# trifectatechfoundation/zlib-rs

Hardware: NVIDIA H100
Metric: deflate_level6_raw_input_throughput_silesia_small_tar (higher is better)
Workload: dtype u8

## Files before the change

zlib_rs_b200/csrc/zb_engine.cu:

```cuda
#include <cuda_runtime.h>
#include <stdio.h>
#include <stdlib.h>
#include <string.h>
#include <algorithm>
#include <cassert>
#include <new>
#include "../../include/zb_engine.h"
#include "zb_kernels.cuh"
#include "zb_engine_internal.h"

namespace zb {

constexpr uint32_t kSlowSub9 = 24576;
constexpr uint32_t kTailTiles = 2;
constexpr uint32_t kTailSub = 512;

thread_local char g_err[256] = "";

static void set_err(const char *what, cudaError_t e)
{
    snprintf(g_err, sizeof g_err, "%s: %s", what, cudaGetErrorString(e));
}

#define CK(call)                                                  \
    do {                                                          \
        cudaError_t e_ = (call);                                  \
        if (e_ != cudaSuccess) { set_err(#call, e_); return ZB_E_CUDA; } \
    } while (0)

__global__ void k_match(JobBufs);
__global__ void k_skip(JobBufs, uint32_t);
__global__ void k_skip_walk(JobBufs);
__global__ void k_nxt(JobBufs);
__global__ void k_path_tiles(JobBufs);
__global__ void k_path_chain(JobBufs, uint32_t, uint32_t);
__global__ void k_path_groups(JobBufs, uint32_t, uint32_t, uint4 *, uint32_t *);
__global__ void k_path_chain2(JobBufs, uint32_t, uint32_t, const uint4 *, uint32_t *, uint32_t *);
__global__ void k_path_mark(JobBufs, const uint32_t *, const uint32_t *);
__global__ void k_iter_lists(JobBufs, uint32_t *, uint32_t *, uint32_t);
__global__ void k_emit(JobBufs);
__global__ void k_holes(JobBufs, uint32_t);
__global__ void k_holes_cmp(JobBufs, uint32_t, uint32_t);
__global__ void k_tail(JobBufs);
__global__ void k_block_hist(JobBufs, uint32_t *);
__global__ void k_build_blocks(JobBufs, const uint32_t *);
__global__ void k_scan_blocks(JobBufs);
__global__ void k_encode(JobBufs);
__global__ void k_finish(JobBufs, const uint32_t *);
__global__ void k_literal_syms(JobBufs);
__global__ void k_stored(JobBufs);
__global__ void k_links2_std(JobBufs, uint32_t);
__global__ void k_links2_roll(JobBufs, uint32_t);
__global__ void k_links_fix_std(JobBufs);
__global__ void k_links_fix_roll(JobBufs);
__global__ void k_slow(JobBufs);
__global__ void k_rle(JobBufs);
__global__ void k_emit_slow(JobBufs);
__global__ void k_tail_slow(JobBufs);
__global__ void k_serial_low(JobBufs);
__global__ void k_links_dict_ghost(JobBufs, uint32_t *);
__global__ void k_links_dict_ghost_apply(JobBufs, const uint32_t *);
__global__ void k_bgzf_setup(BgzfJob, uint64_t);
__global__ void k_serial_low_members(JobBufs, BgzfJob);
__global__ void k_bgzf_medium(JobBufs, BgzfJob);
__global__ void k_bgzf_slow_steps(JobBufs, BgzfJob);
__global__ void k_bgzf_slow_walk(JobBufs, BgzfJob);
__global__ void k_bgzf_rle_steps(JobBufs, BgzfJob);
__global__ void k_bgzf_literals(JobBufs, BgzfJob);
__global__ void k_bgzf_hist(JobBufs, BgzfJob, uint32_t *);
__global__ void k_bgzf_build(JobBufs, BgzfJob, const uint32_t *);
__global__ void k_bgzf_size(JobBufs, BgzfJob);
__global__ void k_bgzf_scan(JobBufs, BgzfJob);
__global__ void k_bgzf_encode(JobBufs, BgzfJob);
__global__ void k_bgzf_frame(JobBufs, BgzfJob);
__global__ void k_batch_stage(const uint8_t *, const uint64_t *, const uint8_t *, const uint64_t *, BgzfJob, uint8_t *, uint64_t);
__global__ void k_batch_dict_ghost(JobBufs, BgzfJob);
__global__ void k_flush_blocks(JobBufs, BgzfJob);
__global__ void k_deflate_points(JobBufs, BgzfJob, IdxWriteJob);

constexpr uint32_t kMatchSmemBytes = (kWSize + kMatchSub + 512) + (kWSize + kMatchSub) * 2 + ((kWSize + kMatchSub) / 32 + 1) * 4 * 4 + 8192;
constexpr uint32_t kPathSmemBytes = kPathTile * 4 * 3;
constexpr uint32_t kLinks2SmemBytes = 65536 * 2 + kLinkTile * 2 + kLinkTile + 64 + 2048;
constexpr uint32_t kSkipSmemBytes = 2 * kWSize * 2 + 2 * (2 * kWSize / 32) * 4 + 8192 + 64;
constexpr uint32_t kSkipWalkSmemBytes = (kWSize + kSkipSlice) * 2 + (kWSize + kSkipSlice) / 32 * 4 + 8192;
constexpr uint32_t kSlowSubMax = 24576;
constexpr uint32_t kSlowSmemBytes = (kWSize + kSlowSubMax + kSlowAhead) * 3;
constexpr uint32_t kChainSmemBytes = kChainChunkTiles * kPathHead * 8;
constexpr uint32_t kChain2MaxSmem = 200 * 1024;
constexpr uint32_t kSerialSmemBytes = (65536 + kWSize) * 2 + 35824 + 16;
constexpr uint32_t kSerialSmemQuick = 65536 * 2 + 65536 + 16;

int Engine::init(int dev)
{
    int n = 0;
    cudaError_t e = cudaGetDeviceCount(&n);
    if (e != cudaSuccess || n == 0) {
        snprintf(g_err, sizeof g_err, "no CUDA device (%s)", e == cudaSuccess ? "count 0" : cudaGetErrorString(e));
        return ZB_E_NODEVICE;
    }
    if (dev < 0 || dev >= n) { snprintf(g_err, sizeof g_err, "device %d out of range", dev); return ZB_E_PARAM; }
    device = dev;
    CK(cudaSetDevice(dev));
    CK(cudaStreamCreateWithFlags(&st, cudaStreamNonBlocking));
    CK(cudaStreamCreateWithFlags(&st2, cudaStreamNonBlocking));
    CK(cudaEventCreateWithFlags(&evf, cudaEventDisableTiming));
    CK(cudaEventCreateWithFlags(&evt, cudaEventDisableTiming));
    for (int i = 0; i < kUpChunks; i++) CK(cudaEventCreateWithFlags(&evc[i], cudaEventDisableTiming));
    CK(cudaEventCreateWithFlags(&evk, cudaEventDisableTiming));
    CK(cudaEventCreate(&ev0));
    CK(cudaEventCreate(&ev1));
    CK(upload_tables());
    CK(cudaFuncSetAttribute(k_match, cudaFuncAttributeMaxDynamicSharedMemorySize, kMatchSmemBytes));
    CK(cudaFuncSetAttribute(k_skip, cudaFuncAttributeMaxDynamicSharedMemorySize, kSkipSmemBytes));
    CK(cudaFuncSetAttribute(k_skip_walk, cudaFuncAttributeMaxDynamicSharedMemorySize, kSkipWalkSmemBytes));
    CK(cudaFuncSetAttribute(k_links2_std, cudaFuncAttributeMaxDynamicSharedMemorySize, kLinks2SmemBytes));
    CK(cudaFuncSetAttribute(k_links2_roll, cudaFuncAttributeMaxDynamicSharedMemorySize, kLinks2SmemBytes));
    CK(cudaFuncSetAttribute(k_slow, cudaFuncAttributeMaxDynamicSharedMemorySize, kSlowSmemBytes));
    CK(cudaFuncSetAttribute(k_path_tiles, cudaFuncAttributeMaxDynamicSharedMemorySize, kPathSmemBytes));
    CK(cudaFuncSetAttribute(k_path_mark, cudaFuncAttributeMaxDynamicSharedMemorySize, kPathSmemBytes));
    CK(cudaFuncSetAttribute(k_path_chain, cudaFuncAttributeMaxDynamicSharedMemorySize, kChainSmemBytes));
    CK(cudaFuncSetAttribute(k_path_groups, cudaFuncAttributeMaxDynamicSharedMemorySize, kChain2MaxSmem));
    CK(cudaFuncSetAttribute(k_path_chain2, cudaFuncAttributeMaxDynamicSharedMemorySize, kChain2MaxSmem));
    CK(cudaFuncSetAttribute(k_serial_low, cudaFuncAttributeMaxDynamicSharedMemorySize, kSerialSmemBytes));
    CK(cudaFuncSetAttribute(k_serial_low_members, cudaFuncAttributeMaxDynamicSharedMemorySize, kSerialSmemBytes));
    CK(cudaMallocHost(&h_info, sizeof(JobInfo)));
    CK(cudaMalloc(&d_info, sizeof(JobInfo)));
    CK(cudaMalloc(&d_check, 16));
    { int rc_ = inflate_init(); if (rc_ != ZB_OK) return rc_; }
    return ZB_OK;
}

Engine::~Engine()
{
    if (device < 0) return;
    cudaSetDevice(device);
    for (auto &b : bufs) if (b.p) cudaFree(b.p);
    if (h_stage) cudaFreeHost(h_stage);
    if (h_info) cudaFreeHost(h_info);
    if (d_info) cudaFree(d_info);
    if (d_check) cudaFree(d_check);
    if (ev0) cudaEventDestroy(ev0);
    if (ev1) cudaEventDestroy(ev1);
    if (evf) cudaEventDestroy(evf);
    if (evt) cudaEventDestroy(evt);
    for (int i = 0; i < kUpChunks; i++) if (evc[i]) cudaEventDestroy(evc[i]);
    if (evk) cudaEventDestroy(evk);
    if (st2) cudaStreamDestroy(st2);
    if (st) cudaStreamDestroy(st);
}

void Engine::pbegin()
{
    if (!profile) return;
    if (!pev0) { cudaEventCreate(&pev0); cudaEventCreate(&pev1); }
    cudaEventRecord(pev0, st);
}

void Engine::pend(int phase, uint32_t nlaunch)
{
    if (!profile) return;
    cudaEventRecord(pev1, st);
    cudaEventSynchronize(pev1);
    float ms = 0;
    cudaEventElapsedTime(&ms, pev0, pev1);
    phase_ms[phase] += ms;
    phase_launches[phase] += nlaunch;
}

int Engine::reserve(int slot, size_t bytes, void **out)
{
    Buf &b = bufs[slot];
    if (b.cap < bytes) {
        if (b.p) { cudaFree(b.p); b.p = nullptr; b.cap = 0; }
        size_t want = bytes + (bytes >> 3) + 4096;
        cudaError_t e = cudaMalloc(&b.p, want);
        if (e != cudaSuccess) { set_err("cudaMalloc", e); return ZB_E_MEM; }
        b.cap = want;
    }
    *out = b.p;
    return ZB_OK;
}

int Engine::stage(size_t bytes)
{
    if (h_stage_cap < bytes) {
        if (h_stage) cudaFreeHost(h_stage);
        h_stage = nullptr;
        h_stage_cap = 0;
        cudaError_t e = cudaMallocHost(&h_stage, bytes + (bytes >> 3) + 4096);
        if (e != cudaSuccess) { set_err("cudaMallocHost", e); return ZB_E_MEM; }
        h_stage_cap = bytes + (bytes >> 3) + 4096;
    }
    return ZB_OK;
}


size_t deflate_bound(size_t n) { return (size_t)stream_bound(n); }

int Engine::deflate(const void *src, size_t n_in, bool src_dev, void *dst, size_t dst_cap, bool dst_dev, int level, int strategy,
                    int window_bits, uint32_t flags, zb_deflate_result *res, const void *dict, size_t dict_len, IdxWrite *iw)
{
    if (flags & ZB_FLAG_BGZF) {
        const uint32_t ml = (flags >> 8) & 15u;
        if ((flags & ~(ZB_FLAG_BGZF | ZB_FLAG_MEMLEVEL(15))) || (ml && ml != 8) || dict_len || window_bits != 31 || strategy != 0 ||
            level < -1 || level > 9) {
            snprintf(g_err, sizeof g_err, "ZB_FLAG_BGZF takes window_bits 31, Z_DEFAULT_STRATEGY, level -1..9 and no other flag");
            return ZB_E_PARAM;
        }
        return deflate_bgzf(src, n_in, src_dev, dst, dst_cap, dst_dev, level, res, iw);
    }
    size_t dstart = 0;
    if (dict_len) {
        if (!dict || window_bits >= 0) { snprintf(g_err, sizeof g_err, "a dictionary needs a raw stream (the caller frames FDICT / DICTID)"); return ZB_E_PARAM; }
        if (dict_len >= 2 * (size_t)kWSize) { dict = static_cast<const uint8_t *>(dict) + (dict_len - kWSize); dict_len = kWSize; }
        dstart = dict_len;
    }
    const size_t n = n_in + dstart;
    int mem_level = (int)((flags >> 8) & 15u);
    if (mem_level == 0) mem_level = 8;
    if (mem_level > 9) return ZB_E_PARAM;
    if (!res || (!src && n) || !dst) return ZB_E_PARAM;
    memset(res, 0, sizeof *res);
    if (n > 0xF0000000ull) { snprintf(g_err, sizeof g_err, "input too large for one job (%zu)", n); return ZB_E_PARAM; }
    if (level == -1) level = 6;
    if (level < 0 || level > 9 || strategy < 0 || strategy > 4) return ZB_E_PARAM;
    uint32_t wrap;
    if (window_bits < 0) { if (window_bits < -15 || window_bits > -8) return ZB_E_PARAM; wrap = 0; }
    else if (window_bits > 15) { if (window_bits < 24 || window_bits > 31) return ZB_E_PARAM; wrap = 2; }
    else { if (window_bits < 8) return ZB_E_PARAM; wrap = 1; }
    const int wb = window_bits < 0 ? -window_bits : window_bits > 15 ? window_bits - 16 : window_bits;
    CK(cudaSetDevice(device));
    const uint32_t N = (uint32_t)n;
    launches = 0;

    JobBufs jb;
    memset(&jb, 0, sizeof jb);
    int rc;
    void *p;
    const size_t npad = (size_t)N + kPad;
    const uint32_t nwords = (N >> 5) + 2;
    const uint32_t nmt = N / kMatchTile + 1, npt = N / kPathTile + 1;
    const bool low_parallel = (flags & ZB_FLAG_LOW_PARALLEL) != 0 || dstart != 0;
    const bool serial_low = (level == 1 || level == 2) && strategy != 2 && strategy != 3 && !low_parallel;
    const uint32_t block_syms = (serial_low && level == 1) ? kBlockSyms : (1u << (mem_level + 6)) - 1u;
    const uint32_t max_blocks = N / block_syms + 2;
    const size_t out_cap = (deflate_bound(n) + 15) & ~(size_t)15;
    if ((rc = stage((size_t)nmt + 64 + ((size_t)N / 512 + 2 + npt + nmt + 8) * 4 + 64)) != ZB_OK) return rc;
    uint8_t *h_dirty = static_cast<uint8_t *>(h_stage);
    uint32_t *h_lists = reinterpret_cast<uint32_t *>(static_cast<uint8_t *>(h_stage) + (((size_t)nmt + 64 + 15) & ~(size_t)15));
#define RES(slot, bytes, field, type)                                   \
    if ((rc = reserve(slot, bytes, &p)) != ZB_OK) return rc;            \
    jb.field = static_cast<type>(p);
    uint8_t *d_in;
    if ((rc = reserve(S_IN, npad + 16, &p)) != ZB_OK) return rc;
    d_in = static_cast<uint8_t *>(p);
    jb.in = d_in;
    jb.N = N;
    jb.start = (uint32_t)dstart;
    jb.nmt = nmt;
    jb.tail_start = N > 2 * kTailZone ? N - kTailZone : 0;
    jb.block_syms = block_syms;
    jb.serial_mode = serial_low ? (uint32_t)level : 0u;
    RES(S_L, npad * 2, L, uint16_t *)
    RES(S_SK, npad * 2, SK, uint16_t *)
    RES(S_HOLES, (size_t)nwords * 4, holes, uint32_t *)
    RES(S_HOLESN, (size_t)nwords * 4, holes_new, uint32_t *)
    RES(S_M, npad * 4, M, uint32_t *)
    RES(S_NXT, ((size_t)N + 16) * 4, nxt, uint32_t *)
    RES(S_PEXIT, ((size_t)N + 16) * 4, pexit, uint32_t *)
    RES(S_PCNT, ((size_t)N + 16) * 4, pcnt, uint32_t *)
    RES(S_SYMIDX, ((size_t)N + 16) * 4, symidx, uint32_t *)
    RES(S_PHEAD, (size_t)npt * kPathHead * 8, phead, uint2 *)
    RES(S_TENTRY, (size_t)npt * 4, tile_entry, uint32_t *)
    RES(S_TSYMB, (size_t)npt * 4, tile_symbase, uint32_t *)
    RES(S_MARKN, (size_t)npt + 16, mark_needed, uint8_t *)
    const uint32_t nlists = npt * (kPathTile / kPathSub);
    RES(S_LLIST, (size_t)nlists * kLongPerSub * 4, long_list, uint32_t *)
    RES(S_LCNT, (size_t)nlists * 4, long_cnt, uint32_t *)
    RES(S_TDIRTY, 2 * ((size_t)nmt + 16), tile_dirty, uint8_t *)
    jb.skip_fall = jb.tile_dirty + nmt + 16;
    RES(S_SYMS, ((size_t)N + 64) * sizeof(Sym), syms, Sym *)
    RES(S_SYMB, 40000 * 4, sym_base, uint32_t *)
    RES(S_BMAP, (size_t)nmt * 8192, bucket_map, uint32_t *)
    RES(S_LR, npad * 2, Lr, uint16_t *)
    RES(S_KEYS, npad * 2, keys, uint16_t *)
    RES(S_LLAST, (size_t)nmt * 65536 * 2, link_last, uint16_t *)
    RES(S_CSTATE, (size_t)(npt + 1) * 16, chain_state, uint4 *)
    uint32_t chainG = 16;
    while ((uint64_t)chainG * chainG < npt) chainG += 8;
    const uint32_t chain_groups = (npt + chainG - 1) / chainG;
    const uint32_t chain2_smem = chainG * kPathHead * 8 + chain_groups * kPathHead * 16 + chainG * 8;
    const bool chain2 = chain2_smem <= kChain2MaxSmem;
    if ((rc = reserve(S_GFN, (size_t)chain_groups * kPathHead * 16 + ((size_t)npt + 4) * 4, &p)) != ZB_OK) return rc;
    uint4 *d_gfn = static_cast<uint4 *>(p);
    uint32_t *d_mark_cnt = reinterpret_cast<uint32_t *>(d_gfn + (size_t)chain_groups * kPathHead);
    uint32_t *d_mark_list = d_mark_cnt + 4;
    auto launch_chain = [&](uint32_t first_tile) {
        if (chain2) {
            k_path_groups<<<chain_groups, 1024, chainG * kPathHead * 8, st>>>(jb, npt, chainG, d_gfn, d_mark_cnt);
            k_path_chain2<<<chain_groups, 1024, chain2_smem, st>>>(jb, npt, chainG, d_gfn, d_mark_list, d_mark_cnt);
            launches++;
        } else k_path_chain<<<1, 1024, kChainSmemBytes, st>>>(jb, npt, first_tile);
    };
    auto launch_mark = [&](uint32_t grid) {
        if (chain2) k_path_mark<<<grid < npt ? grid : npt, 1024, kPathSmemBytes, st>>>(jb, d_mark_list, d_mark_cnt);
        else k_path_mark<<<npt, 1024, kPathSmemBytes, st>>>(jb, nullptr, nullptr);
    };
    uint32_t *d_lists;
    const uint32_t max_list = N / 512 + 2;
    if ((rc = reserve(S_LISTS, ((size_t)max_list + npt + nmt + 8) * 4, &p)) != ZB_OK) return rc;
    d_lists = static_cast<uint32_t *>(p);
    RES(S_HDIFF, (size_t)nwords * 8, hdiff, uint32_t *)
    jb.hdiff_words = nwords;
    RES(S_HCOARSE, (size_t)(N >> 10) + 16, hcoarse, uint8_t *)
    RES(S_MCHG, (((size_t)N >> 8) + 16) * 4 + 64, mchg, uint8_t *)
    RES(S_BLOCKS, (size_t)max_blocks * sizeof(BlockDesc), blocks, BlockDesc *)
    RES(S_BBASE, (size_t)max_blocks * 4, block_base, uint32_t *)
    uint32_t *d_freq;
    if ((rc = reserve(S_FREQ, (size_t)max_blocks * 320 * 4, &p)) != ZB_OK) return rc;
    d_freq = static_cast<uint32_t *>(p);
    uint8_t *d_out;
    if (dst_dev && dst_cap >= out_cap) d_out = static_cast<uint8_t *>(dst);
    else { if ((rc = reserve(S_OUT, out_cap + 16, &p)) != ZB_OK) return rc; d_out = static_cast<uint8_t *>(p); }
    jb.out = d_out;
    jb.out_cap = out_cap;
    void *d_ck;
    const size_t ck_bytes = ((size_t)N / 16384 + 16) * 8;
    if ((rc = reserve(S_CK, ck_bytes, &d_ck)) != ZB_OK) return rc;
#undef RES
    jb.info = d_info;
    jb.level = (uint32_t)level;
    jb.strategy_fixed = strategy == 4;
    const bool lf_zero = strategy >= 2;
    jb.wrap = wrap;
    jb.hdr_len = wrap == 1 ? 2 : wrap == 2 ? 10 : 0;
    jb.huffman_only = strategy == 2 && level != 0;
    jb.not_last = (flags & ZB_FLAG_NOT_LAST) ? 1 : 0;
    jb.end_mode = (flags & ZB_FLAG_END_PARTIAL) ? 1u : (flags & ZB_FLAG_END_BLOCK) ? 2u : 0u;
    jb.prime_bits = (flags >> 12) & 7u;
    if ((jb.end_mode && !jb.not_last) || (jb.prime_bits && wrap != 0)) { snprintf(g_err, sizeof g_err, "END_* needs NOT_LAST, PRIME a raw stream"); return ZB_E_PARAM; }
    if (jb.not_last && (level == 0 || wrap != 0)) { snprintf(g_err, sizeof g_err, "NOT_LAST needs raw deflate and level > 0"); return ZB_E_PARAM; }
    jb.xfl = gzip_xfl(level, strategy);
    int eng_level = level;
    const int wb_eff = wb == 8 ? 9 : wb;
    const bool small_ok = wb_eff < 15 && (uint64_t)N + kMinLookahead <= (1ull << wb_eff);
    bool exact = (wb_eff == 15 || small_ok) && (dstart == 0 || wb_eff == 15);
    jb.cinfo = small_ok ? (uint32_t)(wb_eff - 8) : 7u;
    jb.wsize = kWSize;
    const bool serial_win = wb_eff < 15 && !small_ok && N <= 32000u && level >= 3 && level <= 6 && strategy != 2 && strategy != 3;
    if (serial_win) {
        jb.wsize = 1u << wb_eff;
        jb.cinfo = (uint32_t)(wb_eff - 8);
        jb.tail_start = 0;
        exact = true;
    }
    const bool par_win = wb_eff < 15 && !small_ok && !serial_win && level >= 3 && level <= 6 && strategy != 2 && strategy != 3 && dstart == 0;
    if (par_win) {
        jb.wsize = 1u << wb_eff;
        jb.cinfo = (uint32_t)(wb_eff - 8);
        exact = true;
    }
    const bool slow_win = wb_eff < 15 && !small_ok && dstart == 0 && level != 0 && ((level >= 7 && strategy != 2) || strategy == 3);
    if (slow_win) {
        jb.wsize = 1u << wb_eff;
        jb.cinfo = (uint32_t)(wb_eff - 8);
        exact = true;
    }
    if (wb_eff < 15 && (level == 0 || (strategy == 2 && level != 0) || serial_low)) {
        jb.wsize = 1u << wb_eff;
        jb.cinfo = (uint32_t)(wb_eff - 8);
        exact = true;
    }
    if (level != 0 && !jb.huffman_only) {
        if (level < 3 && !serial_low) { eng_level = 3; exact = exact && strategy == 3; }
        if (strategy == 3) jb.slow_mode = 2;
        else if (level > 6) { jb.slow_mode = 1; jb.sp = slow_params(level); jb.sp.filtered = strategy == 1; jb.sp.wsize = jb.wsize; }
    }
    if (jb.slow_mode) jb.tail_start = N;
    jb.lp = level_params(eng_level);
    if (level != 0 && !jb.huffman_only) jb.level = (uint32_t)level;
    if (lf_zero && !jb.strategy_fixed && !jb.huffman_only) jb.level = 1;

    CK(cudaEventRecord(ev0, st));
    if (profile) { for (int i = 0; i < kPhases; i++) { phase_ms[i] = 0; phase_launches[i] = 0; } }
    uint32_t up_chunks = 0;
    size_t up_len[kUpChunks] = {0};
    const bool chunked_upload = !src_dev && !dstart && n_in >= ((size_t)4 << 20) && level != 0 && !jb.huffman_only &&
                                !jb.serial_mode && jb.slow_mode != 2;
    if (chunked_upload) {
        size_t chunk = ((n_in + kUpChunks - 1) / kUpChunks + kLinkTile - 1) / kLinkTile * kLinkTile;
        if (chunk < (size_t)device_sm_count() * kLinkTile) chunk = (size_t)device_sm_count() * kLinkTile;
        CK(cudaStreamWaitEvent(st2, ev0, 0));
        for (size_t off = 0; off < n_in; off += chunk) {
            const size_t len = n_in - off < chunk ? n_in - off : chunk;
            CK(cudaMemcpyAsync(d_in + off, static_cast<const uint8_t *>(src) + off, len, cudaMemcpyHostToDevice, st2));
            if (off + len == n_in) CK(cudaMemsetAsync(d_in + n, 0, kPad, st2));
            CK(cudaEventRecord(evc[up_chunks], st2));
            up_len[up_chunks++] = off + len;
        }
    } else {
        pbegin();
        if (dstart) CK(cudaMemcpyAsync(d_in, dict, dstart, src_dev ? cudaMemcpyDefault : cudaMemcpyHostToDevice, st));
        if (n_in) CK(cudaMemcpyAsync(d_in + dstart, src, n_in, src_dev ? cudaMemcpyDeviceToDevice : cudaMemcpyHostToDevice, st));
        CK(cudaMemsetAsync(d_in + n, 0, kPad, st));
        pend(9, 0);
    }
    CK(cudaMemsetAsync(d_info, 0, sizeof(JobInfo), st));
    CK(cudaMemsetAsync(d_out, 0, out_cap, st));
    if (jb.prime_bits) {
        h_prime = (uint8_t)((flags >> 16) & ((1u << jb.prime_bits) - 1u));
        CK(cudaMemcpyAsync(d_out, &h_prime, 1, cudaMemcpyHostToDevice, st));
    }
    cudaStream_t st_ck = chunked_upload ? st2 : st;
    pbegin();
    if (wrap == 1 || (wrap == 0 && (flags & ZB_FLAG_CHECK_ADLER))) { CK(launch_adler32(d_in + dstart, n_in, 1, d_ck, ck_bytes, d_check, st_ck)); launches += 2; }
    else if (wrap == 2 || (wrap == 0 && (flags & ZB_FLAG_CHECK_CRC))) { CK(launch_crc32(d_in + dstart, n_in, 0, d_ck, ck_bytes, d_check, st_ck)); launches += 2; }
    else CK(cudaMemsetAsync(d_check, 0, 4, st_ck));
    if (chunked_upload) CK(cudaEventRecord(evk, st2));
    pend(8, 2);

    auto links_tiles = [&](bool roll) {
        uint32_t t_done = 0;
        for (uint32_t k = 0; k < (chunked_upload ? up_chunks : 1u); k++) {
            uint32_t t_hi = nmt;
            if (chunked_upload) {
                cudaStreamWaitEvent(st, evc[k], 0);
                if (k + 1 < up_chunks) t_hi = up_len[k] >= 64 ? (uint32_t)((up_len[k] - 64) / kLinkTile) : 0;
            }
            if (t_hi <= t_done) continue;
            if (roll) k_links2_roll<<<t_hi - t_done, 1024, kLinks2SmemBytes, st>>>(jb, t_done);
            else k_links2_std<<<t_hi - t_done, 1024, kLinks2SmemBytes, st>>>(jb, t_done);
            if (k) launches++;
            t_done = t_hi;
        }
        if (chunked_upload) cudaStreamWaitEvent(st, evk, 0);
    };
    uint32_t iters = 0;
    if (level == 0) {
        const uint32_t nb = n_in == 0 ? 1 : (uint32_t)((n_in + 65534) / 65535);
        k_stored<<<nb, 256, 0, st>>>(jb);
        launches++;
        k_finish<<<1, 32, 0, st>>>(jb, d_check);
        launches++;
    } else {
        if (jb.huffman_only) {
            k_literal_syms<<<(uint32_t)(n_in / 256 + 1), 256, 0, st>>>(jb);
            launches++;
        } else if (jb.serial_mode) {
            iters = 1;
            pbegin();
            k_serial_low<<<1, 32, jb.serial_mode == 2 ? kSerialSmemBytes : kSerialSmemQuick, st>>>(jb);
            launches++;
            pend(1, 1);
        } else {
            CK(cudaMemsetAsync(jb.holes, 0, (size_t)nwords * 4, st));
            CK(cudaMemsetAsync(jb.holes_new, 0, (size_t)nwords * 4, st));
            CK(cudaMemsetAsync(jb.tile_dirty, 1, nmt, st));
            CK(cudaMemsetAsync(jb.skip_fall, 0, nmt, st));
            CK(cudaMemsetAsync(jb.tile_entry, 0xee, (size_t)npt * 4, st));
            CK(cudaMemsetAsync(jb.M + N, 0, (size_t)kPad * 4, st));
            CK(cudaMemsetAsync(jb.L + N, 0, (size_t)kPad * 2, st));
            pbegin();
            if (jb.slow_mode == 2) {
            } else if (jb.slow_mode && jb.sp.slow) {
                links_tiles(true);
                k_links_fix_roll<<<N / 256 + 1, 256, 0, st>>>(jb);
                launches += 2;
            } else {
                links_tiles(false);
                k_links_fix_std<<<N / 256 + 1, 256, 0, st>>>(jb);
                launches += 2;
                if (dstart >= 3 && n_in) {
                    uint32_t *d_first = reinterpret_cast<uint32_t *>(d_check) + 2;
                    CK(cudaMemsetAsync(d_first, 0xff, 4, st));
                    k_links_dict_ghost<<<(kMaxDist + 255) / 256, 256, 0, st>>>(jb, d_first);
                    k_links_dict_ghost_apply<<<1, 32, 0, st>>>(jb, d_first);
                    launches += 2;
                }
            }
            if (!jb.slow_mode) CK(cudaMemcpyAsync(jb.Lr, jb.L, npad * 2, cudaMemcpyDeviceToDevice, st));
            pend(0, 1);
            if (jb.slow_mode) {
                if (n_in > 0) {
                    iters = 1;
                    pbegin();
                    if (jb.slow_mode == 2) k_rle<<<(N + 255) / 256, 256, 0, st>>>(jb);
                    else {
                        jb.match_sub = level >= 9 ? kSlowSub9 : level == 8 ? 4096u : 8192u;
                        k_slow<<<(N + jb.match_sub - 1) / jb.match_sub, 1024, (kWSize + jb.match_sub + kSlowAhead) * 3, st>>>(jb);
                    }
                    pend(1, 1);
                    if (profile) phase_ms[11] = phase_ms[1];
                    pbegin();
                    k_path_tiles<<<npt, 1024, kPathSmemBytes, st>>>(jb);
                    launch_chain(0);
                    launch_mark(npt);
                    pend(3, 3);
                    pbegin();
                    k_emit_slow<<<(N + 255) / 256, 256, 0, st>>>(jb);
                    pend(4, 1);
                    launches += 5;
                }
                pbegin();
                k_tail_slow<<<1, 32, 0, st>>>(jb);
                launches++;
                pend(5, 1);
            } else {
            if (jb.tail_start > 0) {
                uint32_t n_dirty = nmt;
                for (;;) {
                    iters++;
                    uint32_t mthreads = 1024;
                    if (iters == 1) jb.match_sub = 4096;
                    else if (n_dirty <= kTailTiles) { jb.match_sub = kTailSub; mthreads = 256; }
                    else {
                        const uint64_t per_cta = (uint64_t)n_dirty * kMatchTile / (4 * (uint64_t)device_sm_count());
                        jb.match_sub = per_cta >= 8192 ? 8192 : per_cta >= 4096 ? 4096 : per_cta >= 2048 ? 2048 : 1024;
                    }
                    uint32_t nsub = (N + jb.match_sub - 1) / jb.match_sub;
                    uint32_t n_ptiles = npt, first_ptile = 0;
                    jb.skip_list = nullptr;
                    jb.nxt_list = nullptr;
                    if (iters > 1) {
                        jb.skip_list = d_lists;
                        jb.nxt_list = d_lists + nmt + 8;
                        n_ptiles = h_info->n_ptiles ? h_info->n_ptiles : 1;
                        first_ptile = h_info->first_ptile;
                        nsub = (n_dirty ? n_dirty : 1) * (kMatchTile / jb.match_sub);
                        if (n_dirty > kSkipWalkTiles) {
                            pbegin();
                            k_skip<<<n_dirty, 1024, kSkipSmemBytes, st>>>(jb, 0);
                            pend(1, 1);
                            launches++;
                        } else if (n_dirty) {
                            pbegin();
                            k_skip_walk<<<n_dirty * (kMatchTile / kSkipSlice), 1024, kSkipWalkSmemBytes, st>>>(jb);
                            k_skip<<<n_dirty, 1024, kSkipSmemBytes, st>>>(jb, 1);
                            pend(1, 2);
                            launches += 2;
                        }
                    }
                    const uint32_t msmem = (kWSize + jb.match_sub + 512) + (kWSize + jb.match_sub) * 2 +
                                           (iters > 1 ? ((kWSize + jb.match_sub) / 32 + 1) * 4 * 4 + 8192 : 64);
                    jb.use_bucket_map = iters > 1;
                    pbegin();
                    k_match<<<nsub, mthreads, msmem, st>>>(jb);
                    pend(1, 1);
                    if (profile && iters == 1) phase_ms[11] = phase_ms[1];
                    pbegin();
                    k_nxt<<<n_ptiles * (kPathTile / 1024), 1024, 0, st>>>(jb);
                    pend(2, 1);
                    pbegin();
                    k_path_tiles<<<n_ptiles, 1024, kPathSmemBytes, st>>>(jb);
                    launch_chain(first_ptile);
                    launch_mark(iters == 1 ? npt : 2 * n_ptiles + 16);
                    pend(3, 3);
                    pbegin();
                    k_holes<<<(nlists * kLongPerSub + 255) / 256, 256, 0, st>>>(jb, nlists);
                    k_holes_cmp<<<(nwords + 255) / 256, 256, 0, st>>>(jb, nwords, nmt);
                    pend(4, 2);
                    launches += 7;
                    k_iter_lists<<<1, 1024, 0, st>>>(jb, d_lists, d_lists + nmt + 8, npt);
                    launches++;
                    CK(cudaMemcpyAsync(h_info, d_info, sizeof(JobInfo), cudaMemcpyDeviceToHost, st));
                    CK(cudaStreamSynchronize(st));
                    if (h_info->error) { snprintf(g_err, sizeof g_err, "engine error flags 0x%x (parse)", h_info->error); return ZB_E_INTERNAL; }
                    if (getenv("ZB_DEBUG")) {
                        static unsigned long long last[3];
                        if (iters == 1) memset(last, 0, sizeof last);
                        const double ctas = (double)(h_info->dbg[0] - last[0]) + 1e-9;
                        fprintf(stderr, "iter %u dirty %u: ctas %llu stage %.1f walk %.1f kcyc/cta, holes_changed %u, sub %u first_tile %u chain %u\n",
                                iters, n_dirty, h_info->dbg[0] - last[0], (h_info->dbg[1] - last[1]) / 1e3 / ctas,
                                (h_info->dbg[2] - last[2]) / 1e3 / ctas, h_info->holes_changed, jb.match_sub, first_ptile, chain2 ? 2u : 1u);
                        memcpy(last, h_info->dbg, sizeof last);
                    }
                    if (!h_info->holes_changed) break;
                    n_dirty = h_info->n_dirty;
                    if (iters > N / 257u + 4096u) { snprintf(g_err, sizeof g_err, "hole iteration did not converge"); return ZB_E_INTERNAL; }
                }
            }
            CK(cudaEventRecord(evf, st));
            CK(cudaStreamWaitEvent(st2, evf, 0));
            k_tail<<<1, 32, 0, st2>>>(jb);
            launches++;
            CK(cudaEventRecord(evt, st2));
            if (jb.tail_start > 0) {
                pbegin();
                k_emit<<<(jb.tail_start + 255) / 256, 256, 0, st>>>(jb);
                launches++;
                pend(4, 1);
            }
            pbegin();
            CK(cudaStreamWaitEvent(st, evt, 0));
            pend(5, 1);
            }
        }
        CK(cudaMemcpyAsync(h_info, d_info, sizeof(JobInfo), cudaMemcpyDeviceToHost, st));
        CK(cudaStreamSynchronize(st));
        if (h_info->error) { snprintf(g_err, sizeof g_err, "engine error flags 0x%x (tail)", h_info->error); return ZB_E_INTERNAL; }
        const uint32_t nblocks = h_info->n_blocks;
        if (nblocks == 0 || nblocks > max_blocks) { snprintf(g_err, sizeof g_err, "bad block count %u", nblocks); return ZB_E_INTERNAL; }
        pbegin();
        k_block_hist<<<nblocks, 256, 0, st>>>(jb, d_freq);
        k_build_blocks<<<nblocks, 32, 0, st>>>(jb, d_freq);
        k_scan_blocks<<<1, 256, 0, st>>>(jb);
        pend(6, 3);
        pbegin();
        k_encode<<<nblocks, 1024, 0, st>>>(jb);
        k_finish<<<1, 32, 0, st>>>(jb, d_check);
        pend(7, 2);
        launches += 5;
    }
    CK(cudaMemcpyAsync(h_info, d_info, sizeof(JobInfo), cudaMemcpyDeviceToHost, st));
    CK(cudaStreamSynchronize(st));
    CK(cudaGetLastError());
    if (h_info->error) {
        if (h_info->error & 8u) return ZB_E_BUF;
        snprintf(g_err, sizeof g_err, "engine error flags 0x%x (encode)", h_info->error);
        return ZB_E_INTERNAL;
    }
    const uint64_t out_bytes = h_info->out_bytes;
    if (out_bytes > dst_cap) {
        res->out_bytes = out_bytes;
        return ZB_E_BUF;
    }
    if (iw) {
        IdxWriteJob w{iw->span, zbi_targets(n, iw->span), n, 1, 0, level == 0 ? 1u : 0u, 0, nullptr, nullptr};
        const IdxHeader h{kIdxMagic, kIdxVersion, iw->span, n, out_bytes, wrap ? h_info->adler : 1u, wrap == 0 ? -15 : wrap == 1 ? 15 : 31,
                          0, 0, 0};
        BgzfJob bj;
        memset(&bj, 0, sizeof bj);
        if ((rc = index_written(jb, bj, w, h, iw)) != ZB_OK) return rc;
    }
    if (d_out != dst) {
        pbegin();
        CK(cudaMemcpyAsync(dst, d_out, out_bytes, dst_dev ? cudaMemcpyDeviceToDevice : cudaMemcpyDeviceToHost, st));
        pend(10, 0);
    }
    CK(cudaEventRecord(ev1, st));
    CK(cudaStreamSynchronize(st));
    float ms = 0;
    CK(cudaEventElapsedTime(&ms, ev0, ev1));
    res->out_bytes = out_bytes;
    res->check = h_info->adler;
    res->data_type = (int32_t)h_info->data_type;
    res->iterations = iters;
    res->n_symbols = h_info->n_syms;
    res->n_blocks = h_info->n_blocks;
    res->gpu_launches = launches;
    res->exact_parity = exact ? 1 : 0;
    res->gpu_ms = ms;
    res->bits_used = (uint32_t)(h_info->total_bits & 7u) ? (uint32_t)(h_info->total_bits & 7u) : 8u;
    if (jb.not_last && jb.end_mode && (h_info->total_bits & 7u)) {
        uint8_t last = 0;
        CK(cudaMemcpy(&last, d_out + out_bytes, 1, cudaMemcpyDeviceToHost));
        res->carry = last & ((1u << (h_info->total_bits & 7u)) - 1u);
    }
    return ZB_OK;
}

MemberClasses MemberClasses::uniform(int level, uint32_t nm, uint32_t N)
{
    MemberParams mp;
    batch_member_params(level, 0 , 15, 8, 0, &mp);
    MemberClasses mc;
    mc.level = level;
    mc.nslots = level > 0 ? nm * kBgzfMaxBlocks : 0u;
    for (uint32_t c = mp.cls + 1; c <= kClasses; c++) {
        mc.beg[c] = nm;
        mc.off[c] = N;
    }
    return mc;
}

int Engine::members_alloc(JobBufs &jb, BgzfJob &bj, const MemberClasses &mc, uint32_t nm, uint32_t S, size_t span, size_t out_cap,
                          uint32_t wrap, uint32_t **d_freq)
{
    const uint32_t nmt = S / kLinkTile + 1, nslots = mc.nslots;
    memset(&jb, 0, sizeof jb);
    bj = BgzfJob{};
    int rc;
    void *p;
#define RES(slot, bytes, field, type)                                   \
    if ((rc = reserve(slot, bytes, &p)) != ZB_OK) return rc;            \
    jb.field = static_cast<type>(p);
    RES(S_IN, span + kPad + 16, in, const uint8_t *)
    jb.N = S;
    jb.wsize = kWSize;
    RES(S_OUT, out_cap + 16, out, uint8_t *)
    jb.out_cap = out_cap;
    *d_freq = nullptr;
    if (nslots) {
        RES(S_SYMS, (span + 64) * sizeof(Sym), syms, Sym *)
        RES(S_BLOCKS, (size_t)nslots * sizeof(BlockDesc), blocks, BlockDesc *)
        RES(S_BBASE, (size_t)nslots * 4, block_base, uint32_t *)
        if ((rc = reserve(S_FREQ, (size_t)nslots * 320 * 4, &p)) != ZB_OK) return rc;
        *d_freq = static_cast<uint32_t *>(p);
    }
    if (mc.any(kClassMedium, kClassRle)) {
        RES(S_L, (span + kPad) * 2, L, uint16_t *)
        RES(S_KEYS, (span + kPad) * 2, keys, uint16_t *)
        RES(S_LLAST, (size_t)nmt * 65536 * 2, link_last, uint16_t *)
    }
    if (mc.any(kClassSlow, kClassHuff)) {
        RES(S_M, span * 4, M, uint32_t *)
        RES(S_NXT, span * 4, nxt, uint32_t *)
    }
#undef RES
    const size_t m8 = ((size_t)nm * 8 + 15) & ~(size_t)15, m4 = ((size_t)nm * 4 + 15) & ~(size_t)15;
    const size_t mi_bytes = ((size_t)nm * sizeof(JobInfo) + 15) & ~(size_t)15;
    if ((rc = reserve(S_BGZF, 2 * m8 + 4 * m4 + mi_bytes + sizeof(BgzfCtl), &p)) != ZB_OK) return rc;
    uint8_t *t = static_cast<uint8_t *>(p);
    bj.nm = nm;
    bj.wrap = wrap;
    bj.moff = reinterpret_cast<uint64_t *>(t);
    bj.mout = reinterpret_cast<uint64_t *>(t + m8);
    bj.mlen = reinterpret_cast<uint32_t *>(t + 2 * m8);
    bj.mcheck = reinterpret_cast<uint32_t *>(t + 2 * m8 + m4);
    bj.mbytes = reinterpret_cast<uint32_t *>(t + 2 * m8 + 2 * m4);
    bj.mstored = reinterpret_cast<uint32_t *>(t + 2 * m8 + 3 * m4);
    bj.minfo = reinterpret_cast<JobInfo *>(t + 2 * m8 + 4 * m4);
    bj.ctl = reinterpret_cast<BgzfCtl *>(t + 2 * m8 + 4 * m4 + mi_bytes);
    if (mc.level >= 0) {
        const int level = mc.level;
        jb.level = (uint32_t)level;
        jb.block_syms = kBlockSyms;
        jb.serial_mode = level == 1 || level == 2 ? (uint32_t)level : 0u;
        if (level >= 3 && level <= 6) jb.lp = level_params(level);
        if (level >= 7) { jb.slow_mode = 1; jb.sp = slow_params(level); jb.sp.wsize = kWSize; }
    }
    return ZB_OK;
}

static size_t result_bytes(const BgzfJob &bj)
{
    return reinterpret_cast<const uint8_t *>(bj.ctl + 1) - reinterpret_cast<const uint8_t *>(bj.minfo);
}

int Engine::members_stage(const JobBufs &jb, const BgzfJob &bj, const uint64_t *h_moff, const uint32_t *h_mlen, const uint64_t *h_soff,
                          uint64_t *d_soff, size_t n_soff, const void *src, bool src_dev, uint64_t base, uint64_t total, uint8_t *d_copy,
                          const uint8_t *d_dict, const uint64_t *d_mdsrc)
{
    const uint32_t nm = bj.nm;
    CK(cudaMemcpyAsync(bj.moff, h_moff, (size_t)nm * 8, cudaMemcpyHostToDevice, st));
    CK(cudaMemcpyAsync(bj.mlen, h_mlen, (size_t)nm * 4, cudaMemcpyHostToDevice, st));
    CK(cudaMemcpyAsync(d_soff, h_soff, n_soff * 8, cudaMemcpyHostToDevice, st));
    if (!src_dev && total) CK(cudaMemcpyAsync(d_copy, static_cast<const uint8_t *>(src) + base, total, cudaMemcpyHostToDevice, st));
    const uint8_t *d_src = src_dev ? static_cast<const uint8_t *>(src) + base : d_copy;
    k_batch_stage<<<nm, 256, 0, st>>>(d_src + (h_soff[0] - base), d_soff, d_dict, d_mdsrc, bj, const_cast<uint8_t *>(jb.in), jb.N);
    CK(cudaMemsetAsync(const_cast<uint8_t *>(jb.in) + jb.N, 0, kPad + 16, st));
    CK(cudaMemsetAsync(bj.minfo, 0, result_bytes(bj), st));
    CK(cudaMemsetAsync(jb.out, 0, jb.out_cap, st));
    launches++;
    return ZB_OK;
}

void Engine::members_parse(const JobBufs &jb, const BgzfJob &bj, const MemberClasses &mc, bool ghost)
{
    auto links = [&](uint32_t c0, uint32_t c1, bool roll) {
        if (!mc.any(c0, c1)) return false;
        JobBufs r = jb;
        r.in += mc.off[c0];
        r.L += mc.off[c0];
        r.keys += mc.off[c0];
        r.N = (uint32_t)(mc.off[c1] - mc.off[c0]);
        const uint32_t nt = r.N / kLinkTile + 1;
        if (roll) {
            k_links2_roll<<<nt, 1024, kLinks2SmemBytes, st>>>(r, 0);
            k_links_fix_roll<<<r.N / 256 + 1, 256, 0, st>>>(r);
        } else {
            k_links2_std<<<nt, 1024, kLinks2SmemBytes, st>>>(r, 0);
            k_links_fix_std<<<r.N / 256 + 1, 256, 0, st>>>(r);
        }
        launches += 2;
        return true;
    };
    auto view = [&](uint32_t c0, uint32_t c1) {
        const uint32_t m0 = mc.beg[c0];
        assert(m0 == 0 || bj.mslot);
        const auto at = [m0](auto *t) { return t ? t + m0 : t; };
        BgzfJob v = bj;
        v.nm = mc.beg[c1] - m0;
        v.moff = at(v.moff);
        v.mlen = at(v.mlen);
        v.minfo = at(v.minfo);
        v.mp = at(v.mp);
        v.mslot = at(v.mslot);
        v.mps = at(v.mps);
        v.mdx = at(v.mdx);
        return v;
    };
    if (links(kClassMedium, kClassSlow9, false) && ghost) {
        const BgzfJob v = view(kClassMedium, kClassSlow9);
        k_batch_dict_ghost<<<v.nm, 256, 0, st>>>(jb, v);
        launches++;
    }
    links(kClassSlow9, kClassRle, true);
    if (mc.any(kClassQuick, kClassQuick + 1)) {
        JobBufs q = jb;
        q.serial_mode = 1;
        const BgzfJob v = view(kClassQuick, kClassQuick + 1);
        k_serial_low_members<<<v.nm, 32, kSerialSmemQuick, st>>>(q, v);
        launches++;
    }
    if (mc.any(kClassFast, kClassFast + 1)) {
        JobBufs q = jb;
        q.serial_mode = 2;
        const BgzfJob v = view(kClassFast, kClassFast + 1);
        k_serial_low_members<<<v.nm, 32, kSerialSmemBytes, st>>>(q, v);
        launches++;
    }
    if (mc.any(kClassMedium, kClassMedium + 1)) {
        const BgzfJob v = view(kClassMedium, kClassMedium + 1);
        k_bgzf_medium<<<v.nm, 32, 0, st>>>(jb, v);
        launches++;
    }
    if (mc.any(kClassSlow, kClassRle)) {
        const BgzfJob v = view(kClassSlow, kClassRle);
        k_bgzf_slow_steps<<<v.nm * (kMemberMax / 256), 256, 0, st>>>(jb, v);
        k_bgzf_slow_walk<<<(v.nm + 31) / 32, 32, 0, st>>>(jb, v);
        launches += 2;
    }
    if (mc.any(kClassRle, kClassRle + 1)) {
        const BgzfJob v = view(kClassRle, kClassRle + 1);
        k_bgzf_rle_steps<<<v.nm * (kMemberMax / 256), 256, 0, st>>>(jb, v);
        k_bgzf_slow_walk<<<(v.nm + 31) / 32, 32, 0, st>>>(jb, v);
        launches += 2;
    }
    if (mc.any(kClassHuff, kClassHuff + 1)) {
        const BgzfJob v = view(kClassHuff, kClassHuff + 1);
        k_bgzf_literals<<<v.nm * (kMemberMax / 256), 256, 0, st>>>(jb, v);
        launches++;
    }
    if (bj.flushed && mc.any(kClassFast, kClasses)) { k_flush_blocks<<<bj.nm / 256 + 1, 256, 0, st>>>(jb, bj); launches++; }
}

int Engine::members_blocks(JobBufs &jb, BgzfJob &bj, uint32_t nslots, uint32_t *d_freq)
{
    const uint32_t nm = bj.nm;
    if (nslots) {
        k_bgzf_hist<<<nslots, 256, 0, st>>>(jb, bj, d_freq);
        k_bgzf_build<<<nslots, 32, 0, st>>>(jb, bj, d_freq);
        launches += 2;
    }
    k_bgzf_size<<<nm / 256 + 1, 256, 0, st>>>(jb, bj);
    k_bgzf_scan<<<1, 1024, 0, st>>>(jb, bj);
    launches += 2;
    if (nslots) {
        k_bgzf_encode<<<nslots, 1024, 0, st>>>(jb, bj);
        launches++;
    }
    k_bgzf_frame<<<nm + 1, 256, 0, st>>>(jb, bj);
    launches++;
    CK(cudaGetLastError());
    return ZB_OK;
}

int Engine::members_finish(const char *name, const JobBufs &jb, const BgzfJob &bj, BgzfCtl *h_ctl, std::initializer_list<Readback> back,
                           void *dst, size_t dst_cap, bool dst_dev, zb_deflate_result *res, const std::function<int(uint64_t)> &before_copy)
{
    CK(cudaMemcpyAsync(h_ctl, bj.ctl, sizeof(BgzfCtl), cudaMemcpyDeviceToHost, st));
    for (const Readback &b : back)
// ... 984 lines not shown
```

zlib_rs_b200/csrc/zb_engine_internal.h:

```cpp
#pragma once
#include <cuda_runtime.h>
#include <stddef.h>
#include <stdint.h>
#include <functional>
#include <initializer_list>
#include <vector>
#include "../../include/zb_engine.h"
#include "zb_index.h"
#include "zb_zip.h"
#include "zb_kernels.cuh"

namespace zb {

extern thread_local char g_err[256];
size_t deflate_bound(size_t n);

enum { S_IN, S_L, S_HOLES, S_HOLESN, S_M, S_NXT, S_PEXIT, S_PCNT, S_SYMIDX, S_TENTRY, S_TSYMB, S_TDIRTY, S_SYMS, S_SYMB,
       S_BLOCKS, S_SCRATCH, S_FREQ, S_OUT, S_CK, S_INF0, S_INF1, S_PHEAD, S_SK, S_MARKN, S_LLIST, S_LCNT, S_BMAP, S_HDIFF, S_HCOARSE, S_CSTATE, S_LISTS, S_LR, S_LLAST, S_BBASE, S_MCHG, S_GFN, S_KEYS, S_SHARD,
       S_MEMT, S_MEMC,
       S_BGZF,
       S_BATCH,
       S_INDEX,
       S_INDEXW,
       S_AUTO,
       S_ZIPIN,
       S_ZIPPAY,
       S_ZIPOUT,
       S_ZIPTAB,
       S_COUNT };

struct ShardState {
    int phase = 0;
    JobBufs jb;
    uint32_t off = 0, S = 0, E = 0, total = 0;
    uint32_t bs = 0, npt = 0, O = 0, n = 0, blo = 0, nloc = 0;
    bool is_last = false, tables = false;
    uint4 *gfn = nullptr;
    uint32_t chainG = 0, chain_groups = 0, chain2_smem = 0;
    uint32_t freq_lo[320], freq_hi[320];
    zb_shard_span span;
};

struct IdxBlock {
    uint64_t start_bit, out_off;
    uint32_t out_len, type;
};
struct TraceMember {
    IdxMember m;
    std::vector<IdxBlock> blocks;
};
struct InfTrace {
    std::vector<TraceMember> members;
    std::vector<IdxBlock> blocks;
    uint32_t kind = 0;
};
struct IdxBuild {
    uint64_t span = 0;
    InfTrace tr;
    zb_index *out = nullptr;
};
struct IdxWrite {
    uint64_t span = 0;
    zb_index *out = nullptr;
};

struct Carve {
    uint8_t *base = nullptr;
    size_t used = 0;
    template <class T> T *take(size_t n)
    {
        T *p = base ? reinterpret_cast<T *>(base + used) : nullptr;
        used += (n * sizeof(T) + 63) & ~(size_t)63;
        return p;
    }
};

struct MemberClasses {
    int level = -1;
    uint32_t nslots = 0;
    uint32_t beg[kClasses + 1] = {};
    uint64_t off[kClasses + 1] = {};
    bool any(uint32_t c0, uint32_t c1) const { return beg[c1] > beg[c0]; }
    static MemberClasses uniform(int level, uint32_t nm, uint32_t N);
};
struct Readback {
    void *host;
    const void *dev;
    size_t bytes;
};

struct Engine {
    static constexpr int kSlots = 49;
    struct Buf { void *p = nullptr; size_t cap = 0; };
    int device = -1;
    cudaStream_t st = nullptr, st2 = nullptr;
    cudaEvent_t evf = nullptr, evt = nullptr;
    cudaEvent_t ev0 = nullptr, ev1 = nullptr;
    static constexpr int kUpChunks = 8;
    cudaEvent_t evk = nullptr;
    cudaEvent_t evc[kUpChunks] = {nullptr};
    Buf bufs[kSlots];
    void *h_stage = nullptr;
    size_t h_stage_cap = 0;
    JobInfo *h_info = nullptr, *d_info = nullptr;
    uint32_t *d_check = nullptr;
    void *d_inf_state = nullptr, *h_inf_state = nullptr;
    uint32_t launches = 0;
    uint8_t h_prime = 0;
    static constexpr int kPhases = 12;
    bool profile = false;
    float phase_ms[kPhases] = {0};
    uint32_t phase_launches[kPhases] = {0};
    cudaEvent_t pev0 = nullptr, pev1 = nullptr;
    void pbegin();
    void pend(int phase, uint32_t nlaunch);

    int init(int dev);
    int inflate_init();
    ~Engine();
    int reserve(int slot, size_t bytes, void **out);
    int stage(size_t bytes);
    template <class F> int carve(int slot, F &&lay)
    {
        Carve c;
        lay(c);
        void *p = nullptr;
        const int rc = slot < 0 ? stage(c.used) : reserve(slot, c.used, &p);
        if (rc != ZB_OK) return rc;
        c = Carve{static_cast<uint8_t *>(slot < 0 ? h_stage : p)};
        lay(c);
        return ZB_OK;
    }
    int deflate(const void *src, size_t n, bool src_dev, void *dst, size_t dst_cap, bool dst_dev, int level, int strategy,
                int window_bits, uint32_t flags, zb_deflate_result *res, const void *dict = nullptr, size_t dict_len = 0,
                IdxWrite *iw = nullptr);
    int deflate_bgzf(const void *src, size_t n, bool src_dev, void *dst, size_t dst_cap, bool dst_dev, int level, zb_deflate_result *res,
                     IdxWrite *iw = nullptr);
    int index_written(const JobBufs &jb, const BgzfJob &bj, const IdxWriteJob &w, const IdxHeader &h, IdxWrite *iw);
    struct DictTable {
        enum Kind { kNone, kShared, kPerItem } kind = kNone;
        const void *data = nullptr;
        const uint64_t *off = nullptr;
        size_t n = 0;
        const uint32_t *which = nullptr;
    };
    int deflate_batch(const DictTable &dt, const void *src, const uint64_t *src_off, size_t n_items, bool src_dev, void *dst,
                      size_t dst_cap, bool dst_dev, int level, int strategy, int window_bits, uint32_t flags, uint64_t *dst_off,
                      uint32_t *checks, zb_deflate_result *res);
    int deflate_flushed(const void *src, const uint64_t *seg_off, size_t n_segs, bool src_dev, void *dst, size_t dst_cap, bool dst_dev,
                        int level, int strategy, int window_bits, uint32_t flags, uint64_t *restart, zb_deflate_result *res);
    int inflate_flushed(const void *src, size_t src_len, bool src_dev, const uint64_t *restart, size_t n_segs, const uint32_t *which,
                        size_t n_which, void *dst, const uint64_t *dst_off, bool dst_dev, int window_bits, zb_inflate_result *items);
    int members_alloc(JobBufs &jb, BgzfJob &bj, const MemberClasses &mc, uint32_t nm, uint32_t S, size_t span, size_t out_cap,
                      uint32_t wrap, uint32_t **d_freq);
    int members_stage(const JobBufs &jb, const BgzfJob &bj, const uint64_t *h_moff, const uint32_t *h_mlen, const uint64_t *h_soff,
                      uint64_t *d_soff, size_t n_soff, const void *src, bool src_dev, uint64_t base, uint64_t total, uint8_t *d_copy,
                      const uint8_t *d_dict, const uint64_t *d_mdsrc);
    void members_parse(const JobBufs &jb, const BgzfJob &bj, const MemberClasses &mc, bool ghost = false);
    int members_blocks(JobBufs &jb, BgzfJob &bj, uint32_t nslots, uint32_t *d_freq);
    int members_finish(const char *name, const JobBufs &jb, const BgzfJob &bj, BgzfCtl *h_ctl, std::initializer_list<Readback> back,
                       void *dst, size_t dst_cap, bool dst_dev, zb_deflate_result *res,
                       const std::function<int(uint64_t)> &before_copy = nullptr);
    int deflate_batch_params(const void *src, const uint64_t *src_off, size_t n_items, bool src_dev, const zb_batch_params *params,
                             size_t n_params, void *dst, size_t dst_cap, bool dst_dev, uint64_t *dst_off, uint32_t *checks,
                             zb_deflate_result *res);
    int inflate(const void *src, size_t n, bool src_dev, void *dst, size_t dst_cap, bool dst_dev, int window_bits,
                zb_inflate_result *res, uint32_t flags = 0, IdxBuild *ib = nullptr);
    int inflate_stream(const uint8_t *d_src, size_t n, uint8_t *d_dst, size_t dst_cap, int window_bits, uint32_t flags,
                       zb_inflate_result *res, InfTrace *tr = nullptr, const uint64_t *auto_base = nullptr);
    int inflate_members(const uint8_t *d_src, size_t n, uint8_t *d_dst, size_t dst_cap, int window_bits, zb_inflate_result *res,
                        InfTrace *tr = nullptr, bool automatic = false);
    int inflate_auto(const void *src, size_t n, bool src_dev, int window_bits, uint32_t flags, uint64_t max_out, zb_inflate_result *res,
                     const void **out);
    int grow_auto(size_t bytes, size_t keep, uint8_t **out);
    int index_points(const uint8_t *d_src, const uint8_t *d_dst, const zb_inflate_result *res, int window_bits, IdxBuild *ib);
    int index_fill(zb_index &x, std::vector<IdxMember> &&M, std::vector<IdxPoint> &&pts, const IdxHeader &h, const uint8_t *d_src,
                   uint64_t shift);
    int index_bgzf(const void *src, size_t n, bool src_dev, zb_inflate_result *res, zb_index *x);
    int index_extract(const zb_index *x, const void *src, size_t src_len, bool src_dev, const uint64_t *offsets, size_t n_ranges,
                      void *dst, const uint64_t *dst_off, bool dst_dev, zb_inflate_result *items);
    struct BatchAuto {
        uint64_t max_out;
        uint64_t *dst_off;
        const void **out;
    };
    int inflate_batch(const DictTable &dt, const void *src, const uint64_t *src_off, size_t n_items, bool src_dev, void *dst,
                      const uint64_t *dst_off, bool dst_dev, int window_bits, zb_inflate_result *items, const BatchAuto *ba = nullptr);
    int inflate_blocks(const void *src, size_t n, uint64_t start_bit, const void *dict, size_t dict_len, void *dst, size_t dst_cap,
                       int check_kind, uint32_t check_start, zb_inflate_seg *out);
    int checksum(bool crc, uint32_t start, const void *buf, size_t len, bool on_dev, uint32_t *out, float *ms);
    int zip_open(const void *src, size_t n, bool src_dev, zb_inflate_result *res, zb_zip **out);
    int zip_extract(const zb_zip *z, const void *src, size_t src_len, bool src_dev, const uint64_t *which, size_t n_which, void *dst,
                    const uint64_t *dst_off, bool dst_dev, zb_inflate_result *items);
    int zip_write(const void *src, const uint64_t *src_off, size_t n, bool src_dev, const void *names, const uint64_t *name_off, int level,
                  void *dst, size_t dst_cap, bool dst_dev, uint64_t *entry_off, zb_deflate_result *res);
    ShardState shard;
    int shard_parse(const void *src, size_t total, bool src_dev, size_t S, size_t E, int level, int strategy, uint32_t flags,
                    zb_shard_entry *table, uint32_t *adler);
    int shard_symbols(uint32_t entry, uint32_t sym_offset, zb_shard_edge *first, zb_shard_edge *last);
    int shard_size(const zb_shard_edge *all, size_t n, zb_shard_span *span);
    int shard_encode(uint64_t bit_offset, void *dst, size_t cap, bool dst_dev, uint64_t *bytes);
    void shard_chain();
};
static_assert(S_COUNT <= Engine::kSlots, "slots");

}

struct zb_index {
    zb::IdxHeader h;
    std::vector<zb::IdxMember> m;
    std::vector<zb::IdxPoint> p;
    std::vector<uint64_t> woff;
    std::vector<uint8_t> win;
};

struct zb_zip {
    std::vector<zb::zip::Entry> e;
    std::vector<uint8_t> names;
    std::vector<uint64_t> name_off;
    uint64_t src_len = 0, cd_off = 0, cd_size = 0;
};
```

zlib_rs_b200/csrc/zb_kernels.cu:

```cuda
#include "zb_kernels.cuh"

namespace zb {

__constant__ HuffTables c_tab;

cudaError_t upload_tables()
{
    HuffTables t;
    init_tables(t);
    return cudaMemcpyToSymbol(c_tab, &t, sizeof t);
}

struct GAcc {
    const uint8_t *data;
    uint32_t N;
    const uint16_t *L;
    const uint32_t *holes;
    const uint32_t *M;
    uint32_t w = kWSize;
    __device__ __forceinline__ uint32_t byte(uint32_t y) const
    {
        while (y >= N) {
            if (y < 2 * w) return 0;
            y -= w;
// ... 397 lines not shown
        if (m_pend && (__popc(m_pend) >= (int)kBatchCmp || m_walk == 0)) {
            uint32_t len = 0;
            bool resolved = false;
            if (state == LS_PEND) {
                uint32_t pa = dbase + xr + clen, pb = dbase + cr + clen;
#pragma unroll 1
                for (uint32_t k = 0; k < kCmpBurst; k++) {
                    uint32_t a0, a1, b0, b1;
                    sld_u64u(pa, a0, a1);
                    sld_u64u(pb, b0, b1);
                    const uint32_t d0 = a0 ^ b0, d1 = a1 ^ b1;
                    if ((d0 | d1) != 0 || clen + 8 >= kMaxMatch) {
                        len = d0 ? clen + ((__ffs(d0) - 1) >> 3) : d1 ? clen + 4 + ((__ffs(d1) - 1) >> 3) : clen + 8;
                        resolved = true;
                        break;
                    }
                    clen += 8; pa += 8; pb += 8;
                }
            }
            uint32_t m_long = 0;
            if (__popc(m_walk | m_pend) <= kCoopCmp) m_long = __ballot_sync(0xffffffffu, state == LS_PEND && !resolved);
            if (m_long) {
                while (m_long) {
                    const uint32_t src = __ffs(m_long) - 1;
                    m_long &= m_long - 1;
                    const uint32_t cl0 = __shfl_sync(0xffffffffu, clen, src);
                    const uint32_t pa0 = __shfl_sync(0xffffffffu, dbase + xr + clen, src) + 8u * lane;
                    const uint32_t pb0 = __shfl_sync(0xffffffffu, dbase + cr + clen, src) + 8u * lane;
                    uint32_t a0, a1, b0, b1;
                    sld_u64u(pa0, a0, a1);
                    sld_u64u(pb0, b0, b1);
                    const uint32_t d0 = a0 ^ b0, d1 = a1 ^ b1;
                    const uint32_t mm = __ballot_sync(0xffffffffu, (d0 | d1) != 0);
                    const uint32_t first = mm ? __ffs(mm) - 1 : 0u;
                    const uint32_t mine = d0 ? ((__ffs(d0) - 1) >> 3) : 4u + ((__ffs(d1) - 1) >> 3);
                    const uint32_t bo = __shfl_sync(0xffffffffu, mine, first);
                    if (lane == src) { len = mm ? cl0 + 8u * first + bo : cl0 + 256u; resolved = true; }
                }
            }
            if (resolved) {
                if (len > kMaxMatch) len = kMaxMatch;
                state = LS_WALK;
                if (len > best) {
                    best = len;
                    res = (len << 16) | (xr - cr);
                    if (best >= nice) { rd = xr - cr; state = LS_FIN; }
                    else { fbase = dbase + best; xb = sld_u8(fbase + xr); load_xw4(); }
                }
                if (state == LS_WALK) {
                    if (--chain == 0) { rd = (xr - cr) | 0x8000u; state = LS_FIN; }
                    else if (cr < lowr + dn) { rd = 0xffffu; state = LS_FIN; }
                    else cr -= dn;
                }
            }
        }
        if (state == LS_FIN) {
            if (filt && Mout[xr] != res) jb.mchg[(ws + xr) >> 6] = 1;
            Mout[xr] = res; RDout[xr] = (uint16_t)rd; state = LS_IDLE;
        }
        const uint32_t m_idle = __ballot_sync(0xffffffffu, state == LS_IDLE);
        const uint32_t m_busy = __ballot_sync(0xffffffffu, state == LS_WALK || state == LS_PEND);
        if ((m_idle | m_busy) == 0) break;
        if (m_idle == 0) continue;
        if (__popc(m_idle) < (int)kBatch && m_busy != 0) continue;
        {
            uint32_t base = 0;
            const uint32_t leader = __ffs(m_idle) - 1;
            if (lane == leader) base = atomicAdd(s_next, (uint32_t)__popc(m_idle));
            base = __shfl_sync(0xffffffffu, base, leader);
            if (state == LS_IDLE) {
                const uint32_t x = base + __popc(m_idle & ((1u << lane) - 1u));
                if (x >= te) state = LS_DONE;
                else if (x + kMSafe > N) { jb.M[x] = 0; }
                else {
                    xr = x - ws;
                    bool skip = false;
                    if (filt) {
                        const uint32_t h = hash_u32(sld_u32u(dbase + xr));
                        skip = !((sbm[h >> 5] >> (h & 31)) & 1u);
                        if (!skip) {
                            const uint32_t rdo = RDout[xr];
                            const bool on_budget = rdo != 0xffffu && (rdo & 0x8000u);
                            const uint32_t lo = rdo == 0xffffu ? (xr > md ? xr - md : 0u) : xr - (rdo & 0x7fffu);
                            bool redo = DiffMaps::any(dm.del, dm.pdel, lo, xr);
                            if (!redo) {
                                if (on_budget) redo = DiffMaps::any(dm.add, dm.padd, lo, xr);
                                else {
                                    const uint32_t m = Mout[xr];
                                    if (m) { const uint32_t h2 = xr - (m & 0xffffu); redo = (dm.add[h2 >> 5] >> (h2 & 31)) & 1u; }
                                }
                            }
                            if (!redo) redo = sld_u16(lbase + 2 * xr) == md;
                            skip = !redo;
                        }
                    }
                    if (!skip) {
                        const uint32_t d0 = sld_u16(lbase + 2 * xr);
                        lowr = xr > md ? xr - md : 0;
                        if (ws == 0 && lowr == 0) lowr = 1;
                        if (xr < lowr + d0) {
                            if (filt && Mout[xr] != 0) jb.mchg[(ws + xr) >> 6] = 1;
                            Mout[xr] = 0; RDout[xr] = 0xffffu;
                        }
                        else {
                            cr = xr - d0;
                            if (lowr + md == xr) lowr++;
                            best = 2; chain = budget; res = 0;
                            fbase = dbase + 2;
                            xb = sld_u8(fbase + xr);
                            load_xw4();
                            state = LS_WALK;
                        }
                    }
                }
            }
        }
    }
}

__global__ void __launch_bounds__(1024, 2) k_match(JobBufs jb)
{
    extern __shared__ __align__(16) uint8_t smem[];
    __shared__ uint32_t s_next;
    __shared__ __align__(8) unsigned long long s_mbar;
    const uint32_t sub = jb.match_sub;
    const uint32_t per_tile = kMatchTile / sub;
    const uint32_t ts = (jb.skip_list ? jb.skip_list[blockIdx.x / per_tile] * per_tile + blockIdx.x % per_tile : blockIdx.x) * sub;
    if (ts >= jb.N) return;
    {
        const uint32_t t0 = ts / kMatchTile, t1 = (min(ts + sub, jb.N) - 1) / kMatchTile;
        if (!jb.tile_dirty[t0] && !jb.tile_dirty[t1]) return;
    }
    const uint32_t data_bytes = kWSize + sub + 512;
    uint8_t *sdata = smem;
    uint16_t *sL = reinterpret_cast<uint16_t *>(smem + data_bytes);
    uint32_t *sh = reinterpret_cast<uint32_t *>(smem + data_bytes + (kWSize + sub) * 2);
    uint32_t *sbm = sh;
    const uint32_t wmax = (kWSize + sub) / 32 + 1;
    uint32_t *sdel = sbm + 2048, *pdel = sdel + wmax, *sadd = pdel + wmax, *padd = sadd + wmax;
    __shared__ uint32_t s_wsum[32];
    const uint32_t N = jb.N;
    const uint32_t te = min(ts + sub, N);
    const uint32_t ws = ts >= kWSize ? ts - kWSize : 0;
    const uint32_t tid = threadIdx.x, nthr = blockDim.x;
    if (jb.use_bucket_map) {
        const uint32_t mt = ts / kMatchTile;
        const uint32_t *bm1 = jb.bucket_map + (size_t)mt * 2048, *bm0 = mt ? bm1 - 2048 : bm1;
        int hit = 0;
        for (uint32_t x = ts + tid; x < te; x += nthr) {
            const uint8_t *q = jb.in + x;
            const uint32_t h = hash_u32((uint32_t)q[0] | ((uint32_t)q[1] << 8) | ((uint32_t)q[2] << 16) | ((uint32_t)q[3] << 24));
            if (((bm0[h >> 5] | bm1[h >> 5]) >> (h & 31)) & 1u) {
                const uint32_t rd = jb.SK[x];
                const uint32_t lo = rd == 0xffffu ? (x > jb.wsize - kMinLookahead ? x - (jb.wsize - kMinLookahead) : 0u) : x - (rd & 0x7fffu);
                for (uint32_t b = lo >> 10; b <= (x >> 10); b++) hit |= jb.hcoarse[b];
            }
        }
        if (!__syncthreads_or(hit)) return;
        for (uint32_t i = tid; i < 2048; i += nthr) sbm[i] = bm0[i] | bm1[i];
        const uint32_t nwd = (te - ws + 31) / 32;
        const uint32_t per = (nwd + 1 + nthr - 1) / nthr;
        const uint32_t wb = tid * per;
        const uint32_t lane_ = tid & 31, warp_ = tid >> 5;
        for (int which = 0; which < 2; which++) {
            const uint32_t *src = which ? jb.hdiff : jb.hdiff + jb.hdiff_words;
            uint32_t *bits = which ? sadd : sdel, *pre = which ? padd : pdel;
            uint32_t mine = 0;
            for (uint32_t k = 0; k < per; k++) {
                const uint32_t w = wb + k;
                if (w <= nwd) { const uint32_t v = w < nwd ? src[(ws >> 5) + w] : 0u; bits[w] = v; mine += __popc(v); }
            }
            uint32_t incl = mine;
#pragma unroll
            for (int d = 1; d < 32; d <<= 1) {
                const uint32_t t = __shfl_up_sync(0xffffffffu, incl, d);
                if (lane_ >= (uint32_t)d) incl += t;
            }
            __syncthreads();
            if (lane_ == 31) s_wsum[warp_] = incl;
            __syncthreads();
            uint32_t run = incl - mine;
            for (uint32_t k = 0; k < warp_; k++) run += s_wsum[k];
            for (uint32_t k = 0; k < per; k++) {
                const uint32_t w = wb + k;
                if (w <= nwd) { pre[w] = run; run += __popc(bits[w]); }
            }
        }
    }
    if (tid == 0) {
        s_next = ts;
        const uint32_t mb = (uint32_t)__cvta_generic_to_shared(&s_mbar);
        asm volatile("mbarrier.init.shared::cta.b64 [%0], 1;" ::"r"(mb) : "memory");
        asm volatile("fence.proxy.async.shared::cta;" ::: "memory");
    }
    const long long t_0 = clock64();
    __syncthreads();
    {
        uint32_t n16 = (te + 512 - ws + 15) / 16;
        if (n16 > data_bytes / 16) n16 = data_bytes / 16;
        const bool bulk = (reinterpret_cast<uintptr_t>(jb.in) & 15u) == 0;
        if (bulk) {
            if (tid == 0) {
                const uint32_t mb = (uint32_t)__cvta_generic_to_shared(&s_mbar), dsts = (uint32_t)__cvta_generic_to_shared(sdata);
                asm volatile("mbarrier.arrive.expect_tx.shared::cta.b64 _, [%0], %1;" ::"r"(mb), "r"(n16 * 16u) : "memory");
                asm volatile("cp.async.bulk.shared::cluster.global.mbarrier::complete_tx::bytes [%0], [%1], %2, [%3];"
                             ::"r"(dsts), "l"(jb.in + ws), "r"(n16 * 16u), "r"(mb) : "memory");
            }
        } else {
            const uint4 *src = reinterpret_cast<const uint4 *>(jb.in + ws);
            uint4 *dst = reinterpret_cast<uint4 *>(sdata);
            for (uint32_t i = tid; i < n16; i += nthr) dst[i] = src[i];
        }
        const uint32_t nl = (te - ws + 7) / 8;
        const uint4 *ls = reinterpret_cast<const uint4 *>(jb.Lr + ws);
        uint4 *ld = reinterpret_cast<uint4 *>(sL);
        for (uint32_t i = tid; i < nl; i += nthr) {
            uint4 v = ls[i];
            v.x |= __vcmpeq2(v.x, 0u); v.y |= __vcmpeq2(v.y, 0u); v.z |= __vcmpeq2(v.z, 0u); v.w |= __vcmpeq2(v.w, 0u);
            ld[i] = v;
        }
        if (bulk) {
            const uint32_t mb = (uint32_t)__cvta_generic_to_shared(&s_mbar);
            uint32_t done = 0;
            while (!done) {
                asm volatile("{\n.reg .pred p;\nmbarrier.try_wait.parity.shared::cta.b64 p, [%1], 0;\nselp.u32 %0, 1, 0, p;\n}"
                             : "=r"(done) : "r"(mb) : "memory");
            }
        }
    }
    __syncthreads();
    const long long t_1 = clock64();
    const LevelParams lp = jb.lp;
    if (!lp.early_exit) {
        match_tile_fast(jb, sdata, sL, sbm, DiffMaps{sdel, pdel, sadd, padd}, ws, te, &s_next);
        __syncthreads();
        if (tid == 0) {
            const long long t_2 = clock64();
            atomicAdd(&jb.info->dbg[0], 1ull);
            atomicAdd(&jb.info->dbg[1], (unsigned long long)(t_1 - t_0));
            atomicAdd(&jb.info->dbg[2], (unsigned long long)(t_2 - t_1));
        }
        return;
    }
    SAccR a{sdata, sL, ws};
    for (uint32_t x = ts + tid; x < te; x += nthr) {
        uint32_t v = 0;
        if (jb.use_bucket_map && x + 4 <= N) {
            const uint32_t h = hash_u32(a.byte(x) | (a.byte(x + 1) << 8) | (a.byte(x + 2) << 16) | (a.byte(x + 3) << 24));
            if (!((sbm[h >> 5] >> (h & 31)) & 1u)) continue;
        }
        if (x + kMSafe <= N) {
            Match m = jb.wsize == kWSize ? lm_walk(a, x, 0xffffffffu, lp) : lm_walk(a, x, 0xffffffffu, lp, DynWin{jb.wsize});
            if (m.len) v = (m.len << 16) | (x - m.start);
        }
        if (jb.use_bucket_map && jb.M[x] != v) jb.mchg[x >> 6] = 1;
        jb.M[x] = v;
        jb.SK[x] = 0xffffu;
    }
}

constexpr uint32_t kMacroReach = 22016;

__device__ __forceinline__ bool path_tile_dirty(const JobBufs &jb, uint32_t pt)
{
    const uint32_t m0 = (pt * kPathTile) / kMatchTile;
    uint32_t m1 = ((pt + 1) * kPathTile + kMacroReach - 1) / kMatchTile;
    if (m1 >= jb.nmt) m1 = jb.nmt - 1;
    bool d = false;
    for (uint32_t m = m0; m <= m1; m++) d = d || jb.tile_dirty[m];
    return d;
}

__global__ void __launch_bounds__(1024) k_nxt(JobBufs jb)
{
    constexpr uint32_t per = kPathTile / 1024;
    const uint32_t tile = jb.nxt_list ? jb.nxt_list[blockIdx.x / per] : blockIdx.x / per;
    if (!path_tile_dirty(jb, tile)) return;
    const uint32_t p = tile * kPathTile + (blockIdx.x % per) * 1024 + threadIdx.x;
    if (p >= jb.tail_start) return;
    if (jb.use_bucket_map) {
        const uint32_t old = jb.nxt[p];
        const uint32_t b0 = p >> 6, b1 = min(p + (old & 0xffffu), jb.N) >> 6;
        bool chg = false;
        for (uint32_t b = b0; b <= b1; b++) chg = chg || jb.mchg[b];
        if (!chg) return;
    }
    GAcc a{jb.in, jb.N, jb.L, jb.holes, jb.M, jb.wsize};
    const uint32_t long_len = 16 * jb.lp.lazy;
    uint32_t ns = 0, nlong = 0, lpos = 0, llen = 0;
    auto see = [&](const Sym &s) {
        if (s.dist && (uint32_t)s.lc + 3u > long_len) { nlong++; lpos = s.pos; llen = s.lc + 3u; }
    };
    const uint32_t np = jb.wsize == kWSize ? macro_step(a, p, jb.lp, jb.tail_start, see, &ns)
                                           : macro_step(a, p, jb.lp, jb.tail_start, see, &ns, DynWin{jb.wsize});
    const uint32_t delta = np - p;
    if (delta > 0xffffu || ns > 0xffu || delta == 0) atomicOr(&jb.info->error, 1u);
    if (nlong && (nlong != 1 || lpos + llen != np || (jb.lp.early_exit ? lpos != p : (llen != 257u && llen != 258u))))
        atomicOr(&jb.info->error, 16u);
    jb.nxt[p] = (delta & 0xffffu) | ((ns & 0xffu) << 16) | (nlong ? kNxtLong : 0u) | (llen == 258u ? kNxtLong258 : 0u) |
                (np >= jb.tail_start ? kNxtTail : 0u);
}

constexpr uint32_t kStuck = 0x80000000u;
__device__ __forceinline__ void path_subtile(const uint32_t *nx, uint32_t *ex, uint32_t *cn, uint32_t s0, uint32_t s1, uint32_t lane)
{
    for (int32_t b = (int32_t)s1 - 32; b >= (int32_t)s0; b -= 32) {
        const uint32_t p = (uint32_t)b + lane;
        const uint32_t v = nx[p];
        uint32_t t, c;
        if (v & kNxtTail) { t = kStuck | p; c = 0; }
        else { t = p + (v & 0xffffu); c = (v >> 16) & 0xffu; }
#pragma unroll
        for (int r = 0; r < 5; r++) {
            const bool inb = !(t & kStuck) && t < (uint32_t)b + 32u;
            const uint32_t src = inb ? t - (uint32_t)b : lane;
            const uint32_t t2 = __shfl_sync(0xffffffffu, t, src);
            const uint32_t c2 = __shfl_sync(0xffffffffu, c, src);
            if (inb) { t = t2; c += c2; }
        }
        if (!(t & kStuck) && t < s1) { c += cn[t]; t = ex[t]; }
        ex[p] = t;
        cn[p] = c;
        __syncwarp();
    }
}

constexpr uint32_t kPathSmem = kPathTile * 4 * 3;

__device__ __forceinline__ void path_load(const JobBufs &jb, uint32_t tbeg, uint32_t *nx)
{
    const uint4 *src = reinterpret_cast<const uint4 *>(jb.nxt + tbeg);
    uint4 *dst = reinterpret_cast<uint4 *>(nx);
#pragma unroll 4
    for (uint32_t g = threadIdx.x; g < kPathTile / 4; g += blockDim.x) {
        const uint32_t p = tbeg + 4 * g;
        uint4 v;
        if (p + 3 < jb.tail_start) v = src[g];
        else {
            const uint32_t t = kNxtTail | 1u;
            v.x = p < jb.tail_start ? jb.nxt[p] : t;
            v.y = p + 1 < jb.tail_start ? jb.nxt[p + 1] : t;
            v.z = p + 2 < jb.tail_start ? jb.nxt[p + 2] : t;
            v.w = t;
        }
        dst[g] = v;
    }
}

__global__ void __launch_bounds__(1024) k_path_tiles(JobBufs jb)
{
    extern __shared__ __align__(16) uint8_t smem[];
    uint32_t *nx = reinterpret_cast<uint32_t *>(smem);
    uint32_t *ex = nx + kPathTile;
    uint32_t *cn = ex + kPathTile;
    const uint32_t tile = jb.nxt_list ? jb.nxt_list[blockIdx.x] : blockIdx.x;
    const uint32_t tbeg = tile * kPathTile;
    if (!path_tile_dirty(jb, tile)) return;
    path_load(jb, tbeg, nx);
    __syncthreads();
    const uint32_t warp = threadIdx.x >> 5, lane = threadIdx.x & 31;
    constexpr uint32_t kExitSub = 1024, nsub = kPathTile / kExitSub;
    for (uint32_t s = warp; s < nsub; s += blockDim.x / 32) path_subtile(nx, ex, cn, s * kExitSub, (s + 1) * kExitSub, lane);
    __syncthreads();
    for (int32_t j = (int32_t)nsub - 2; j >= 0; j--) {
        for (uint32_t i = threadIdx.x; i < kExitSub; i += blockDim.x) {
            const uint32_t p = (uint32_t)j * kExitSub + i;
            uint32_t t = ex[p];
            if (!(t & kStuck) && t < kPathTile) { cn[p] += cn[t]; ex[p] = ex[t]; }
        }
        __syncthreads();
    }
    for (uint32_t i = threadIdx.x; i < kPathTile; i += blockDim.x) {
        const uint32_t p = tbeg + i;
        const uint32_t t = ex[i];
        const uint32_t xa = (t & kStuck) ? (kStuck | (tbeg + (t & ~kStuck))) : tbeg + t;
        if (p < jb.tail_start) {
            jb.pexit[p] = xa;
            jb.pcnt[p] = cn[i];
        }
        if (i < kPathHead) jb.phead[(size_t)tile * kPathHead + i] = make_uint2(xa, cn[i]);
    }
}

constexpr uint32_t kChainChunk = kChainChunkTiles;
__global__ void __launch_bounds__(1024) k_path_chain(JobBufs jb, uint32_t ntiles, uint32_t first_tile)
{
    extern __shared__ __align__(16) uint8_t smem[];
    uint2 *hd = reinterpret_cast<uint2 *>(smem);
    __shared__ uint32_t s_e, s_base, s_done, s_tail;
    __shared__ uint32_t c_entry[kChainChunk], c_base[kChainChunk];
    if (threadIdx.x == 0) {
        if (first_tile == 0) { s_e = jb.start; s_base = 0; s_done = jb.tail_start == 0; s_tail = jb.start; }
        else { const uint4 v = jb.chain_state[first_tile]; s_e = v.x; s_base = v.y; s_done = v.z; s_tail = v.w; }
    }
    for (uint32_t t = threadIdx.x; t < first_tile; t += blockDim.x) jb.mark_needed[t] = 0;
    __syncthreads();
    for (uint32_t c0 = first_tile; c0 < ntiles; c0 += kChainChunk) {
        const uint32_t nt = min(kChainChunk, ntiles - c0);
        for (uint32_t i = threadIdx.x; i < nt * kPathHead; i += blockDim.x) hd[i] = jb.phead[(size_t)c0 * kPathHead + i];
        __syncthreads();
        if (threadIdx.x == 0) {
            uint32_t e = s_e, base = s_base;
            bool done = s_done != 0;
            uint32_t tail_entry = s_tail;
            for (uint32_t k = 0; k < nt; k++) {
                const uint32_t tbeg = (c0 + k) * kPathTile, tend = tbeg + kPathTile;
                jb.chain_state[c0 + k] = make_uint4(e, base, done ? 1u : 0u, tail_entry);
                c_base[k] = base;
                if (done || e >= tend || e >= jb.tail_start) { c_entry[k] = 0xffffffffu; continue; }
                c_entry[k] = e;
                uint32_t x, c;
                if (e - tbeg < kPathHead) { const uint2 v = hd[k * kPathHead + (e - tbeg)]; x = v.x; c = v.y; }
                else { x = jb.pexit[e]; c = jb.pcnt[e]; }
                base += c;
                if (x & kStuck) { tail_entry = x & ~kStuck; done = true; }
                else e = x;
            }
            s_e = e; s_base = base; s_done = done; s_tail = tail_entry;
        }
        __syncthreads();
        for (uint32_t k = threadIdx.x; k < nt; k += blockDim.x) {
            const uint32_t t = c0 + k;
            jb.tile_symbase[t] = c_base[k];
            jb.mark_needed[t] = (jb.tile_entry[t] != c_entry[k]) || path_tile_dirty(jb, t);
            jb.tile_entry[t] = c_entry[k];
        }
        __syncthreads();
    }
    if (threadIdx.x == 0) {
        uint32_t tail_entry = s_tail;
        if (!s_done) { tail_entry = s_e; if (s_e < jb.tail_start) atomicOr(&jb.info->error, 2u); }
        jb.info->tail_entry = tail_entry;
        jb.info->n_mid_syms = s_base;
    }
}

struct ChainState { uint32_t e, base, done, tail; };

template <bool OUT>
__device__ __forceinline__ void chain_walk_group(const JobBufs &jb, const uint2 *hd, uint32_t t0, uint32_t nt, ChainState &s,
                                                 uint32_t *c_entry, uint32_t *c_base)
{
    for (uint32_t k = 0; k < nt; k++) {
        const uint32_t tbeg = (t0 + k) * kPathTile, tend = tbeg + kPathTile;
        if (OUT) c_base[k] = s.base;
        if (s.done || s.e >= tend || s.e >= jb.tail_start) { if (OUT) c_entry[k] = 0xffffffffu; continue; }
        if (OUT) c_entry[k] = s.e;
        uint32_t x, c;
        if (s.e - tbeg < kPathHead) { const uint2 v = hd[k * kPathHead + (s.e - tbeg)]; x = v.x; c = v.y; }
        else { x = jb.pexit[s.e]; c = jb.pcnt[s.e]; }
        s.base += c;
        if (x & kStuck) { s.tail = x & ~kStuck; s.done = 1; }
        else s.e = x;
    }
}

__device__ __forceinline__ void chain_stage_heads(const JobBufs &jb, uint2 *hd, uint32_t t0, uint32_t nt)
{
    const uint4 *src = reinterpret_cast<const uint4 *>(jb.phead + (size_t)t0 * kPathHead);
    uint4 *dst = reinterpret_cast<uint4 *>(hd);
    for (uint32_t i = threadIdx.x; i < nt * kPathHead / 2; i += blockDim.x) dst[i] = src[i];
}

__global__ void __launch_bounds__(1024) k_path_groups(JobBufs jb, uint32_t ntiles, uint32_t G, uint4 *gfn, uint32_t *mark_cnt)
{
    if (blockIdx.x == 0 && threadIdx.x == 0) *mark_cnt = 0;
    extern __shared__ __align__(16) uint8_t smem[];
    uint2 *hd = reinterpret_cast<uint2 *>(smem);
    const uint32_t t0 = blockIdx.x * G, nt = min(G, ntiles - t0);
    chain_stage_heads(jb, hd, t0, nt);
    __syncthreads();
    if (threadIdx.x < kPathHead) {
        ChainState s{t0 * kPathTile + threadIdx.x, 0u, 0u, 0u};
        chain_walk_group<false>(jb, hd, t0, nt, s, nullptr, nullptr);
        gfn[(size_t)blockIdx.x * kPathHead + threadIdx.x] = make_uint4(s.e, s.base, s.done, s.tail);
    }
}

__global__ void __launch_bounds__(1024) k_path_chain2(JobBufs jb, uint32_t ntiles, uint32_t G, const uint4 *gfn, uint32_t *mark_list,
                                                        uint32_t *mark_cnt)
{
    extern __shared__ __align__(16) uint8_t smem[];
    uint2 *hd = reinterpret_cast<uint2 *>(smem);
    uint4 *sg = reinterpret_cast<uint4 *>(smem + (size_t)G * kPathHead * 8);
    uint32_t *c_entry = reinterpret_cast<uint32_t *>(sg + (size_t)blockIdx.x * kPathHead), *c_base = c_entry + G;
    __shared__ ChainState s_st;
    __shared__ uint32_t s_j;
    const uint32_t g = blockIdx.x;
    for (uint32_t i = threadIdx.x; i < g * kPathHead; i += blockDim.x) sg[i] = gfn[i];
    if (threadIdx.x == 0) { s_st = ChainState{jb.start, 0u, jb.tail_start == 0 ? 1u : 0u, jb.start}; s_j = 0; }
    __syncthreads();
    for (;;) {
        if (threadIdx.x == 0) {
            ChainState s = s_st;
            uint32_t j = s_j;
            for (; j < g; j++) {
                const uint32_t gbeg = j * G * kPathTile;
                if (s.done || s.e >= jb.tail_start || s.e - gbeg >= G * kPathTile) continue;
                if (s.e - gbeg >= kPathHead) break;
                const uint4 f = sg[j * kPathHead + (s.e - gbeg)];
                s.e = f.x; s.base += f.y;
                if (f.z) { s.done = 1; s.tail = f.w; }
            }
            s_st = s; s_j = j;
        }
        __syncthreads();
        const uint32_t j = s_j;
        if (j >= g) break;
        chain_stage_heads(jb, hd, j * G, G);
        __syncthreads();
        if (threadIdx.x == 0) {
            ChainState s = s_st;
            chain_walk_group<false>(jb, hd, j * G, G, s, nullptr, nullptr);
            s_st = s; s_j = j + 1;
        }
        __syncthreads();
    }
    const uint32_t t0 = g * G, nt = min(G, ntiles - t0);
    chain_stage_heads(jb, hd, t0, nt);
    __syncthreads();
    if (threadIdx.x == 0) {
        ChainState s = s_st;
        chain_walk_group<true>(jb, hd, t0, nt, s, c_entry, c_base);
        if (g == gridDim.x - 1) {
            uint32_t tail_entry = s.tail;
            if (!s.done) { tail_entry = s.e; if (s.e < jb.tail_start) atomicOr(&jb.info->error, 2u); }
            jb.info->tail_entry = tail_entry;
            jb.info->n_mid_syms = s.base;
        }
    }
    __syncthreads();
    for (uint32_t k = threadIdx.x; k < nt; k += blockDim.x) {
        const uint32_t t = t0 + k;
        jb.tile_symbase[t] = c_base[k];
        const bool mn = (jb.tile_entry[t] != c_entry[k]) || path_tile_dirty(jb, t);
        jb.mark_needed[t] = mn;
        jb.tile_entry[t] = c_entry[k];
        if (mn) mark_list[atomicAdd(mark_cnt, 1u)] = t;
    }
}

__global__ void __launch_bounds__(1024) k_path_mark(JobBufs jb, const uint32_t *list, const uint32_t *list_cnt)
{
    extern __shared__ __align__(16) uint8_t smem[];
    uint32_t *nx = reinterpret_cast<uint32_t *>(smem);
    uint32_t *ex = nx + kPathTile;
    uint32_t *cn = ex + kPathTile;
    __shared__ uint32_t sub_entry[kPathTile / kPathSub], sub_base[kPathTile / kPathSub];
    constexpr uint32_t nsub = kPathTile / kPathSub;
    const uint32_t count = list ? *list_cnt : gridDim.x;
    for (uint32_t b = blockIdx.x; b < count; b += gridDim.x) {
        const uint32_t tile = list ? list[b] : b;
        const uint32_t tbeg = tile * kPathTile;
        if (!jb.mark_needed[tile]) continue;
        const uint32_t entry = jb.tile_entry[tile];
        if (threadIdx.x < nsub) jb.long_cnt[tile * nsub + threadIdx.x] = 0;
        if (entry == 0xffffffffu) {
            for (uint32_t i = threadIdx.x; i < kPathTile; i += blockDim.x)
                if (tbeg + i < jb.tail_start) jb.symidx[tbeg + i] = 0;
            continue;
        }
        __syncthreads();
        path_load(jb, tbeg, nx);
        __syncthreads();
        const uint32_t warp = threadIdx.x >> 5, lane = threadIdx.x & 31;
        for (uint32_t s = warp; s < nsub; s += blockDim.x / 32) path_subtile(nx, ex, cn, s * kPathSub, (s + 1) * kPathSub, lane);
        __syncthreads();
        if (threadIdx.x == 0) {
            uint32_t cur = entry - tbeg, cbase = 0;
            for (uint32_t j = 0; j < nsub; j++) {
                if (!(cur & kStuck) && cur < (j + 1) * kPathSub) {
                    sub_entry[j] = cur;
                    sub_base[j] = cbase;
                    cbase += cn[cur];
                    cur = ex[cur];
                } else sub_entry[j] = 0xffffffffu;
            }
        }
        __syncthreads();
        for (uint32_t i = threadIdx.x; i < kPathTile; i += blockDim.x) ex[i] = 0;
        __syncthreads();
        if (threadIdx.x < nsub) {
            const uint32_t s = threadIdx.x;
            uint32_t p = sub_entry[s];
            if (p != 0xffffffffu) {
                uint32_t idx = sub_base[s], nlong = 0;
                const uint32_t s1 = (s + 1) * kPathSub;
                uint32_t *ll = jb.long_list + (size_t)(tile * nsub + s) * kLongPerSub;
                while (p < s1) {
                    const uint32_t v = nx[p];
                    if (v & kNxtTail) break;
                    if (v & kNxtLong) {
                        if (nlong < kLongPerSub) ll[nlong++] = tbeg + p;
                        else atomicOr(&jb.info->error, 32u);
                    }
                    ex[p] = idx + 1;
                    idx += (v >> 16) & 0xffu;
                    p += v & 0xffffu;
                }
                jb.long_cnt[tile * nsub + s] = nlong;
            }
        }
        __syncthreads();
        for (uint32_t i = threadIdx.x; i < kPathTile; i += blockDim.x)
            if (tbeg + i < jb.tail_start) jb.symidx[tbeg + i] = ex[i];
    }
}

__global__ void __launch_bounds__(256) k_holes(JobBufs jb, uint32_t nlists)
{
    const uint32_t t = blockIdx.x * blockDim.x + threadIdx.x;
    {
        const uint32_t nthr = gridDim.x * blockDim.x;
        for (uint32_t i = t; i < jb.nmt; i += nthr) jb.tile_dirty[i] = 0;
        for (uint32_t i = t; i < jb.nmt * 512; i += nthr) reinterpret_cast<uint4 *>(jb.bucket_map)[i] = make_uint4(0, 0, 0, 0);
        for (uint32_t i = t; i < (jb.N >> 10) + 16; i += nthr) jb.hcoarse[i] = 0;
        for (uint32_t i = t; i < (jb.N >> 8) + 16; i += nthr) reinterpret_cast<uint32_t *>(jb.mchg)[i] = 0;
        if (t == 0) jb.info->holes_changed = 0;
    }
    const uint32_t list = t / kLongPerSub, slot = t % kLongPerSub;
    if (list >= nlists || slot >= jb.long_cnt[list]) return;
    const uint32_t p = jb.long_list[(size_t)list * kLongPerSub + slot];
    const uint32_t v = jb.nxt[p], delta = v & 0xffffu;
    const uint32_t len = jb.lp.early_exit ? delta : ((v & kNxtLong258) ? 258u : 257u);
    const uint32_t pos = p + delta - len;
    uint32_t y0 = pos + 1, y1 = pos + len - 1;
    uint32_t *hn = jb.holes_new;
    while (y0 < y1) {
        const uint32_t w = y0 >> 5, lo = y0 & 31;
        const uint32_t n = min(32u - lo, y1 - y0);
        const uint32_t mask = (n == 32 ? 0xffffffffu : ((1u << n) - 1u)) << lo;
        atomicOr(&hn[w], mask);
        y0 += n;
    }
}

__global__ void __launch_bounds__(256) k_emit(JobBufs jb)
{
    const uint32_t p = blockIdx.x * blockDim.x + threadIdx.x;
    if (p >= jb.tail_start) return;
    const uint32_t idx = jb.symidx[p];
    if (!idx) return;
    GAcc a{jb.in, jb.N, jb.L, jb.holes, jb.M, jb.wsize};
    uint32_t k = jb.tile_symbase[p / kPathTile] + idx - 1, ns = 0;
    Sym *syms = jb.syms;
    auto put = [&](const Sym &s) { syms[k++] = s; };
    if (jb.wsize == kWSize) macro_step(a, p, jb.lp, jb.tail_start, put, &ns);
    else macro_step(a, p, jb.lp, jb.tail_start, put, &ns, DynWin{jb.wsize});
}

__global__ void __launch_bounds__(256) k_holes_cmp(JobBufs jb, uint32_t nwords, uint32_t nmtiles)
{
    __shared__ uint32_t sb[2048];
    const uint32_t w = blockIdx.x * blockDim.x + threadIdx.x;
    uint32_t a = 0, b = 0;
    if (w < nwords) { a = jb.holes[w]; b = jb.holes_new[w]; }
    const bool changed = a != b;
    if (!__syncthreads_or(changed)) {
        if (w < nwords) { jb.hdiff[w] = 0; jb.hdiff[jb.hdiff_words + w] = 0; jb.holes_new[w] = 0; }
        return;
    }
    for (uint32_t i = threadIdx.x; i < 2048; i += blockDim.x) sb[i] = 0;
    __syncthreads();
    if (w < nwords) {
        jb.hdiff[w] = b & ~a;
        jb.hdiff[jb.hdiff_words + w] = a & ~b;
        if (changed) {
            jb.hcoarse[w >> 5] = 1;
            const uint32_t t = (w * 32) / kMatchTile;
            jb.info->holes_changed = 1u;
            jb.tile_dirty[t] = 1;
            if (t + 1 < nmtiles) jb.tile_dirty[t + 1] = 1;
            jb.holes[w] = b;
            uint32_t diff = a ^ b;
            while (diff) {
                const uint32_t y = w * 32 + (__ffs(diff) - 1);
                diff &= diff - 1;
                if (y + 4 <= jb.N) {
                    const uint8_t *q = jb.in + y;
                    const uint32_t h = hash_u32((uint32_t)q[0] | ((uint32_t)q[1] << 8) | ((uint32_t)q[2] << 16) | ((uint32_t)q[3] << 24));
                    atomicOr(&sb[h >> 5], 1u << (h & 31));
                }
            }
        }
        jb.holes_new[w] = 0;
    }
    __syncthreads();
    uint32_t *bm = jb.bucket_map + (size_t)((blockIdx.x * blockDim.x * 32) / kMatchTile) * 2048;
    for (uint32_t i = threadIdx.x; i < 2048; i += blockDim.x) if (sb[i]) atomicOr(&bm[i], sb[i]);
}

__global__ void __launch_bounds__(1024) k_iter_lists(JobBufs jb, uint32_t *skip_list, uint32_t *path_list, uint32_t npt)
{
    __shared__ uint32_t s_wsum[32], s_total, s_first;
    const uint32_t tid = threadIdx.x, lane = tid & 31, warp = tid >> 5;
    if (tid == 0) s_first = 0xffffffffu;
    uint32_t base = 0;
    for (int which = 0; which < 2; which++) {
        const uint32_t n = which ? npt : jb.nmt;
        uint32_t *out = which ? path_list : skip_list;
        base = 0;
        for (uint32_t c0 = 0; c0 < n; c0 += 1024) {
            const uint32_t i = c0 + tid;
            const bool d = i < n && (which ? path_tile_dirty(jb, i) : jb.tile_dirty[i] != 0);
            const uint32_t m = __ballot_sync(0xffffffffu, d);
            __syncthreads();
            if (lane == 0) s_wsum[warp] = __popc(m);
            __syncthreads();
            if (warp == 0) {
                const uint32_t v = s_wsum[lane];
                uint32_t incl = v;
#pragma unroll
                for (int k = 1; k < 32; k <<= 1) { const uint32_t t = __shfl_up_sync(0xffffffffu, incl, k); if (lane >= (uint32_t)k) incl += t; }
                s_wsum[lane] = incl - v;
                if (lane == 31) s_total = incl;
            }
            __syncthreads();
            if (d) {
                out[base + s_wsum[warp] + __popc(m & ((1u << lane) - 1u))] = i;
                if (which) atomicMin(&s_first, i);
            }
            base += s_total;
        }
        __syncthreads();
        if (tid == 0) {
            if (which) { jb.info->n_ptiles = base; jb.info->first_ptile = s_first == 0xffffffffu ? 0u : s_first; }
            else jb.info->n_dirty = base;
        }
        if (tid == 0 && base == 0) out[0] = 0;
    }
}

struct GAccW {
    GAcc g;
    uint32_t w;
    __device__ __forceinline__ uint32_t byte(uint32_t y) const
    {
        while (y >= g.N) {
            if (y < 2 * w) return 0;
            y -= w;
        }
        return g.data[y];
    }
    __device__ __forceinline__ uint32_t link(uint32_t y) const { return g.link(y); }
    __device__ __forceinline__ bool inserted(uint32_t y) const { return g.inserted(y); }
};

__global__ void __launch_bounds__(32) k_tail(JobBufs jb)
{
    __shared__ uint32_t ins[1024];
    if (threadIdx.x != 0) return;
    GAcc a{jb.in, jb.N, jb.L, jb.holes, jb.M, jb.wsize};
    const uint32_t p0 = max(jb.info->tail_entry, jb.start);
    const uint32_t n_mid = jb.info->n_mid_syms;
    uint32_t k = 0;
    Sym *syms = jb.syms + n_mid;
    uint32_t *sb = jb.sym_base;
    if (jb.N - p0 > 1024u * 32u - 64u) { atomicOr(&jb.info->error, 4u); return; }
    auto emit = [&](const Sym &s, uint32_t B) {
        syms[k] = s;
        sb[k] = B;
        k++;
    };
    uint32_t fb;
    if (jb.wsize == kWSize) fb = serial_medium(a, jb.N, p0, ins, 1024u, jb.lp, emit);
    else fb = serial_medium(GAccW{a, jb.wsize}, jb.N, p0, ins, 1024u, jb.lp, emit, DynWin{jb.wsize});
    jb.info->n_syms = n_mid + k;
    jb.info->final_base = fb;
    jb.info->n_blocks = (n_mid + k) / jb.block_syms + 1;
}

__device__ __forceinline__ uint32_t sym_end(const Sym &s) { return s.pos + (s.dist ? (uint32_t)s.lc + 3u : 1u); }

__device__ __forceinline__ void block_hist_body(const Sym *syms, uint32_t begin, uint32_t count, uint32_t *fb)
{
    __shared__ uint32_t lf[kLCodes], df[kDCodes];
    for (uint32_t i = threadIdx.x; i < kLCodes; i += blockDim.x) lf[i] = 0;
    if (threadIdx.x < kDCodes) df[threadIdx.x] = 0;
    __syncthreads();
    for (uint32_t i = threadIdx.x; i < count; i += blockDim.x) {
        const Sym s = syms[begin + i];
        if (s.dist == 0) atomicAdd(&lf[s.lc], 1u);
        else {
            atomicAdd(&lf[257 + c_tab.length_code[s.lc]], 1u);
            atomicAdd(&df[d_code(c_tab, s.dist - 1u)], 1u);
        }
    }
    __syncthreads();
    for (uint32_t i = threadIdx.x; i < kLCodes; i += blockDim.x) fb[i] = lf[i];
    if (threadIdx.x < kDCodes) fb[kLCodes + threadIdx.x] = df[threadIdx.x];
}

__global__ void __launch_bounds__(256) k_block_hist(JobBufs jb, uint32_t *freq )
{
    const uint32_t b = blockIdx.x;
    const uint32_t nsyms = jb.info->n_syms, nblocks = jb.info->n_blocks;
    const uint32_t begin = b * jb.block_syms;
    const uint32_t count = (b + 1 < nblocks) ? jb.block_syms : nsyms - begin;
    block_hist_body(jb.syms, begin, count, freq + b * 320);
    if (threadIdx.x == 0) {
        BlockDesc &bd = jb.blocks[b];
        const bool last = b + 1 == nblocks;
        bd.sym_begin = begin;
        bd.sym_count = count;
        bd.last = last && !jb.not_last;
        const uint32_t start = begin == 0 ? jb.start : sym_end(jb.syms[begin - 1]);
        const uint32_t end = last ? jb.N : sym_end(jb.syms[begin + count - 1]);
        bd.in_start = start;
        bd.in_len = end - start;
        uint32_t Bf;
        if (last) Bf = jb.info->final_base;
        else {
            const uint32_t li = begin + count - 1, n_mid = jb.info->n_mid_syms;
            if (jb.serial_mode) {
                Bf = jb.serial_mode == 2 ? jb.block_base[b] : 0;
            } else if (jb.huffman_only) {
                const uint32_t q = jb.syms[li].pos, w = jb.wsize;
                Bf = q < 2 * w ? 0 : w * (1 + (q - 2 * w) / w);
            } else if (jb.slow_mode == 2) {
                Bf = base_at(jb.syms[li].pos, jb.N, jb.wsize);
            } else if (jb.slow_mode) {
                Bf = base_at(jb.syms[li].pos + 1, jb.N, jb.wsize);
            } else Bf = li < n_mid ? wbase_w(DynWin{jb.wsize}, jb.syms[li].pos) : jb.sym_base[li - n_mid];
        }
        bd.have_window = start >= Bf;
    }
}

__device__ __forceinline__ uint32_t brev_bits(uint32_t code, uint32_t len) { return __brev(code) >> (32u - len); }

template <int KIND>
__device__ __forceinline__ uint32_t xbits_of(uint32_t n) { return KIND == 0 ? (n >= 257 ? extra_lbits(n - 257) : 0u) : KIND == 1 ? extra_dbits(n) : extra_blbits(n); }

template <int KIND>
__device__ int build_tree_warp(TreeScratch &s, TreeState &st, CtData *tree, uint32_t *sh_cnt )
{
    constexpr int elems = KIND == 0 ? kLCodes : KIND == 1 ? kDCodes : kBlCodes;
    constexpr int max_length = KIND == 2 ? kMaxBlBits : kMaxBits;
    const uint32_t lane = threadIdx.x & 31;
    int heap_len = 0, max_code = -1;
    for (int b0 = 0; b0 < elems; b0 += 32) {
        const int n = b0 + (int)lane;
        const bool nz = n < elems && tree[n].fc != 0;
        const uint32_t m = __ballot_sync(0xffffffffu, nz);
        if (nz) { s.heap[heap_len + 1 + __popc(m & ((1u << lane) - 1u))] = (uint32_t)n; s.depth[n] = 0; }
        else if (n < elems) tree[n].dl = 0;
        heap_len += __popc(m);
        if (m) max_code = b0 + 31 - __clz(m);
    }
    __syncwarp();
    if (heap_len < 2) {
        if (lane == 0) {
            while (heap_len < 2) {
                const int node = max_code < 2 ? ++max_code : 0;
                s.heap[++heap_len] = (uint32_t)node;
                tree[node].fc = 1;
                s.depth[node] = 0;
                st.opt_len--;
                if (KIND == 0) st.static_len -= c_tab.sl_len[node];
                else if (KIND == 1) st.static_len -= 5;
            }
        }
        heap_len = 2;
        max_code = __shfl_sync(0xffffffffu, max_code, 0);
        __syncwarp();
    }
    for (int n = 1 + (int)lane; n <= heap_len; n += 32) s.hk[n] = heap_entry(tree, s.depth, s.heap[n]);
    __syncwarp();
    for (int lvl = 31 - __clz(heap_len / 2); lvl >= 0; lvl--) {
        const int first = 1 << lvl, last = min((2 << lvl) - 1, heap_len / 2);
        for (int k = first + (int)lane; k <= last; k += 32) pqdownheap(s, heap_len, k);
        __syncwarp();
    }
    int heap_max = kHeapSize;
    if (lane == 0) {
        int node = elems;
        do {
            const int n = (int)(s.hk[1] & 0xffffu);
            s.hk[1] = s.hk[heap_len--];
            pqdownheap(s, heap_len, 1);
            const int m = (int)(s.hk[1] & 0xffffu);
            s.heap[--heap_max] = (uint32_t)n;
            s.heap[--heap_max] = (uint32_t)m;
            tree[node].fc = (uint16_t)(tree[n].fc + tree[m].fc);
            s.depth[node] = (uint8_t)((s.depth[n] >= s.depth[m] ? s.depth[n] : s.depth[m]) + 1);
            tree[n].dl = tree[m].dl = (uint16_t)node;
            s.hk[1] = heap_entry(tree, s.depth, (uint32_t)node);
            node++;
            pqdownheap(s, heap_len, 1);
        } while (heap_len >= 2);
        s.heap[--heap_max] = (uint32_t)(s.hk[1] & 0xffffu);
        int overflow = 0;
        tree[s.heap[heap_max]].dl = 0;
        for (int h = heap_max + 1; h < kHeapSize; h++) {
            const int n = (int)s.heap[h];
            int bits = tree[tree[n].dl].dl + 1;
            if (bits > max_length) { bits = max_length; overflow++; }
            tree[n].dl = (uint16_t)bits;
        }
        sh_cnt[0] = (uint32_t)overflow;
    }
    heap_max = __shfl_sync(0xffffffffu, heap_max, 0);
    __syncwarp();
    const int overflow = (int)sh_cnt[0];
    __syncwarp();
    if (lane < 16) sh_cnt[lane] = 0;
    __syncwarp();
    uint64_t opt = 0, stat = 0;
    for (int n = (int)lane; n <= max_code; n += 32) {
        const uint32_t bits = tree[n].dl;
        if (tree[n].fc == 0 || bits == 0) continue;
        atomicAdd(&sh_cnt[bits], 1u);
        const uint32_t xb = xbits_of<KIND>((uint32_t)n);
        const uint64_t f = tree[n].fc;
        opt += f * (uint64_t)(bits + xb);
        if (KIND == 0) stat += f * (uint64_t)(c_tab.sl_len[n] + xb);
        else if (KIND == 1) stat += f * (uint64_t)(5 + xb);
    }
#pragma unroll
    for (int d = 16; d >= 1; d >>= 1) { opt += __shfl_xor_sync(0xffffffffu, opt, d); stat += __shfl_xor_sync(0xffffffffu, stat, d); }
    __syncwarp();
    if (lane == 0) {
        st.opt_len += opt;
        st.static_len += stat;
        if (overflow > 0) {
            int ov = overflow, bits;
            do {
                bits = max_length - 1;
                while (sh_cnt[bits] == 0) bits--;
                sh_cnt[bits]--;
                sh_cnt[bits + 1] += 2;
                sh_cnt[max_length]--;
                ov -= 2;
            } while (ov > 0);
            int h = kHeapSize;
            for (bits = max_length; bits != 0; bits--) {
                int n = (int)sh_cnt[bits];
                while (n != 0) {
                    const int m = (int)s.heap[--h];
                    if (m > max_code) continue;
                    if (tree[m].dl != (uint16_t)bits) {
                        st.opt_len += (uint64_t)bits * tree[m].fc;
                        st.opt_len -= (uint64_t)tree[m].dl * tree[m].fc;
                        tree[m].dl = (uint16_t)bits;
                    }
                    n--;
                }
            }
        }
    }
    __syncwarp();
    uint32_t nc = 0;
    {
        uint32_t code = 0;
        for (uint32_t b = 1; b <= (uint32_t)kMaxBits; b++) { code = (code + sh_cnt[b - 1]) << 1; if (b == lane) nc = code; }
    }
    for (int b0 = 0; b0 <= max_code; b0 += 32) {
        const int n = b0 + (int)lane;
        const uint32_t len = n <= max_code ? tree[n].dl : 0u;
        const uint32_t same = __match_any_sync(0xffffffffu, len);
        const uint32_t rank = __popc(same & ((1u << lane) - 1u));
        const uint32_t base = __shfl_sync(0xffffffffu, nc, len & 31u);
        if (len) tree[n].fc = (uint16_t)brev_bits(base + rank, len);
#pragma unroll 1
        for (uint32_t l = 1; l <= (uint32_t)kMaxBits; l++) {
            const uint32_t cnt = __popc(__ballot_sync(0xffffffffu, len == l));
            if (lane == l) nc += cnt;
        }
    }
    __syncwarp();
    return max_code;
}

struct WordSink {
    uint8_t *buf;
    uint32_t nbits;
    __device__ __forceinline__ void put(uint32_t val, uint32_t len)
    {
        const uint32_t byte = nbits >> 3, sh = nbits & 7u;
        const uint32_t v = (val & ((1u << len) - 1u)) << sh;
        if (sh == 0) buf[byte] = (uint8_t)v; else buf[byte] |= (uint8_t)v;
        if (sh + len > 8) { buf[byte + 1] = (uint8_t)(v >> 8); if (sh + len > 16) buf[byte + 2] = (uint8_t)(v >> 16); }
        nbits += len;
    }
};

__device__ void send_tree_fast(WordSink &o, const CtData *bltree, const CtData *tree, int max_code)
{
    int prevlen = -1, curlen, nextlen = tree[0].dl, count = 0, max_count = 7, min_count = 4;
    if (nextlen == 0) { max_count = 138; min_count = 3; }
    for (int n = 0; n <= max_code; n++) {
        curlen = nextlen;
        nextlen = tree[n + 1].dl;
        if (++count < max_count && curlen == nextlen) continue;
        else if (count < min_count) { do { o.put(bltree[curlen].fc, bltree[curlen].dl); } while (--count != 0); }
        else if (curlen != 0) {
            if (curlen != prevlen) { o.put(bltree[curlen].fc, bltree[curlen].dl); count--; }
            o.put(bltree[16].fc, bltree[16].dl);
            o.put((uint32_t)(count - 3), 2);
        } else if (count <= 10) {
            o.put(bltree[17].fc, bltree[17].dl);
            o.put((uint32_t)(count - 3), 3);
        } else {
            o.put(bltree[18].fc, bltree[18].dl);
            o.put((uint32_t)(count - 11), 7);
        }
        count = 0;
        prevlen = curlen;
        if (nextlen == 0) { max_count = 138; min_count = 3; }
        else if (curlen == nextlen) { max_count = 6; min_count = 3; }
        else { max_count = 7; min_count = 4; }
    }
}

__device__ void build_block_warp(TreeScratch &s, BlockDesc &b, const uint32_t *lfreq, const uint32_t *dfreq, bool have_window,
                                 bool strategy_fixed, uint32_t *sh_cnt, TreeState *sh_st)
{
    const uint32_t lane = threadIdx.x & 31;
    uint64_t opt_lenb = 0, static_lenb = 0;
    int max_blindex = 0, lmax = 0, dmax = 0;
    TreeState &st = *sh_st;
    if (lane == 0) { st = TreeState{0, 0}; b.data_type = 2; b.no_eob = 0; }
    __syncwarp();
    if (b.sym_count == 0) {
        if (lane == 0) st.static_len = 7;
    } else {
        {
            bool black = false, white = false;
            for (uint32_t n = lane; n < 256; n += 32) {
                if (lfreq[n] == 0) continue;
                if (n < 32 && ((0xf3ffc07fu >> n) & 1u)) black = true;
                if (n == 9 || n == 10 || n == 13 || n >= 32) white = true;
// ... 463 lines not shown
```

zlib_rs_b200/csrc/zb_kernels.cuh:

```cuda
#pragma once
#include <cuda_runtime.h>
#include "zb_core.h"
#include "zb_huff.h"
#include "zb_slow.h"
#include "zb_bgzf.h"
#include "zb_index.h"

namespace zb {

constexpr uint32_t kLinkTile = 32768;
constexpr uint32_t kMatchTile = 32768;
constexpr uint32_t kMatchSub = 8192;
constexpr uint32_t kPathTile = 16384;
constexpr uint32_t kPathSub = 256;
constexpr uint32_t kLongPerSub = 4;
constexpr uint32_t kPathHead = 64;
constexpr uint32_t kChainChunkTiles = 320;
constexpr uint32_t kNxtTail = 0x80000000u;
constexpr uint32_t kNxtLong = 0x40000000u;
constexpr uint32_t kNxtLong258 = 0x20000000u;
constexpr uint32_t kSymsPerThread = 16;
constexpr uint32_t kSlowAhead = 1024;
constexpr uint32_t kSkipSlice = 4096;
constexpr uint32_t kSkipWalkHops = 256;
constexpr uint32_t kSkipWalkTiles = 32;

__device__ __forceinline__ uint32_t sld_u8(uint32_t a) { uint32_t v; asm volatile("ld.shared.u8 %0, [%1];" : "=r"(v) : "r"(a)); return v; }
__device__ __forceinline__ uint32_t sld_u16(uint32_t a) { uint32_t v; asm volatile("ld.shared.u16 %0, [%1];" : "=r"(v) : "r"(a)); return v; }
__device__ __forceinline__ uint32_t sld_u32(uint32_t a) { uint32_t v; asm volatile("ld.shared.u32 %0, [%1];" : "=r"(v) : "r"(a)); return v; }
__device__ __forceinline__ uint32_t sld_u32u(uint32_t a)
{
    const uint32_t al = a & ~3u;
    return __funnelshift_r(sld_u32(al), sld_u32(al + 4), (a & 3u) * 8u);
}

struct JobInfo {
    uint32_t n_mid_syms;
    uint32_t tail_entry;
    uint32_t n_syms;
    uint32_t final_base;
    uint32_t holes_changed;
    uint32_t n_dirty, n_ptiles, first_ptile;
    uint32_t n_blocks;
    uint32_t data_type;
    uint32_t error;
    uint64_t total_bits;
    uint64_t out_bytes;
    uint32_t adler;
    uint64_t marker_byte;
    unsigned long long dbg[3];
};

struct JobBufs {
    const uint8_t *in;
    uint32_t N;
    uint32_t start;
    uint32_t tail_start;
    uint16_t *L;
    uint16_t *SK;
    uint32_t *hdiff;
    uint32_t hdiff_words;
    uint8_t *hcoarse;
    uint8_t *mchg;
    uint32_t *holes;
    uint32_t *holes_new;
    uint32_t *M;
    uint32_t *nxt;
    uint32_t *pexit;
    uint32_t *pcnt;
    uint2 *phead;
    uint32_t *symidx;
    uint32_t *tile_entry;
    uint32_t *tile_symbase;
    uint8_t *tile_dirty;
    uint8_t *skip_fall;
    Sym *syms;
    uint32_t *sym_base;
    BlockDesc *blocks;
    TreeScratch *scratch;
    uint8_t *out;
    uint64_t out_cap;
    JobInfo *info;
    LevelParams lp;
    uint32_t level;
    uint32_t strategy_fixed;
    uint32_t wrap;
    uint32_t hdr_len;
    uint32_t xfl;
    uint32_t huffman_only;
    uint32_t match_sub;
    uint32_t nmt;
    uint8_t *mark_needed;
    uint32_t *long_list;
    uint32_t *long_cnt;
    SlowParams sp;
    uint32_t slow_mode;
    uint16_t *link_last;
    uint16_t *Lr;
    uint16_t *keys;
    const uint32_t *skip_list;
    const uint32_t *nxt_list;
    uint4 *chain_state;
    uint32_t *bucket_map;
    uint32_t use_bucket_map;
    uint32_t not_last;
    uint32_t end_mode;
    uint32_t prime_bits;
    uint32_t block_syms;
    uint32_t serial_mode;
    uint32_t *block_base;
    uint32_t wsize;
    uint32_t cinfo;
};

struct BgzfCtl {
    uint32_t count;
    uint32_t error;
    uint32_t n_blocks;
    uint32_t n_syms;
    uint32_t data_type;
    uint32_t pad;
    uint64_t out_bytes;
};
struct BgzfJob {
    uint32_t nm;
    uint32_t wrap;
    uint64_t *moff;
    uint32_t *mlen;
    uint32_t *mcheck;
    uint32_t *mbytes;
    uint64_t *mout;
    uint32_t *mstored;
    JobInfo *minfo;
    BgzfCtl *ctl;
    const uint32_t *mps;
    const uint32_t *mdx;
    const uint32_t *dictid;
    uint32_t flushed;
    uint32_t *fcheck;
    uint32_t isize;
    const MemberParams *mp;
    const uint32_t *mslot;
    const uint32_t *morder;
    uint32_t *mcrc;
    ZB_HD uint32_t slot0(uint32_t m) const { return mslot ? mslot[m] : m * kBgzfMaxBlocks; }
    ZB_HD uint32_t nslots(uint32_t m) const { return mslot ? mslot[m + 1] - mslot[m] : kBgzfMaxBlocks; }
    ZB_HD uint32_t wrap_of(uint32_t m) const { return mp ? mp[m].wrap : wrap; }
    ZB_HD uint32_t pstart_of(uint32_t m) const { return mps ? mps[m] : 0u; }
    ZB_HD bool fdict_of(uint32_t m) const { return mdx && mdx[m] != kDictNone; }
    ZB_HD uint32_t dictid_of(uint32_t m) const { return dictid[mdx[m]]; }
    ZB_HD void slot_member(uint32_t b, uint32_t &m, uint32_t &k) const
    {
        if (!mslot) { m = b / kBgzfMaxBlocks; k = b % kBgzfMaxBlocks; return; }
        uint32_t lo = 0, hi = nm;
        while (hi - lo > 1) {
            const uint32_t mid = (lo + hi) / 2;
            if (mslot[mid] <= b) lo = mid; else hi = mid;
        }
        m = lo;
        k = b - mslot[lo];
    }
};

struct IdxCand {
    uint64_t out_off, bit, hdr_bit;
    uint32_t member, btype, found, pad;
};
struct IdxWriteJob {
    uint64_t span, K;
    uint64_t n;
    uint32_t nm;
    uint32_t bgzf;
    uint32_t stored;
    uint32_t pad;
    IdxCand *cand;
    IdxMember *members;
};

cudaError_t upload_tables();
int device_sm_count();
cudaError_t launch_adler32(const uint8_t *d_buf, uint64_t len, uint32_t start, void *d_scratch, size_t scratch_bytes, uint32_t *d_out,
                           cudaStream_t st);
cudaError_t launch_crc32(const uint8_t *d_buf, uint64_t len, uint32_t start, void *d_scratch, size_t scratch_bytes, uint32_t *d_out,
                         cudaStream_t st);
cudaError_t launch_crc32_segments(const uint8_t *d_buf, const uint64_t *d_off, const uint32_t *d_len, uint32_t nseg, uint32_t *d_crc,
                                  cudaStream_t st);
cudaError_t launch_crc32_join(const uint32_t *d_crc, const uint32_t *d_len, const uint32_t *d_count, uint32_t *d_out, cudaStream_t st);
cudaError_t launch_adler32_join(const uint32_t *d_adler, const uint32_t *d_len, const uint32_t *d_count, uint32_t *d_out, cudaStream_t st);
cudaError_t launch_adler32_segments(const uint8_t *d_buf, const uint64_t *d_off, const uint32_t *d_len, uint32_t nseg, uint32_t *d_adler,
                                    cudaStream_t st);

}
```

zlib_rs_b200/csrc/zb_shard.cu:

```cuda
#include <stdio.h>
#include <string.h>
#include "zb_kernels.cuh"
#include "zb_engine_internal.h"
#include "zb_shard.h"

namespace zb {

__global__ void k_slow(JobBufs);
__global__ void k_links2_std(JobBufs, uint32_t);
__global__ void k_links2_roll(JobBufs, uint32_t);
__global__ void k_links_fix_std(JobBufs);
__global__ void k_links_fix_roll(JobBufs);
__global__ void k_path_tiles(JobBufs);
__global__ void k_path_chain(JobBufs, uint32_t, uint32_t);
__global__ void k_path_groups(JobBufs, uint32_t, uint32_t, uint4 *, uint32_t *);
__global__ void k_path_chain2(JobBufs, uint32_t, uint32_t, const uint4 *, uint32_t *, uint32_t *);
__global__ void k_path_mark(JobBufs, const uint32_t *, const uint32_t *);
__global__ void k_emit_slow(JobBufs);
__global__ void k_tail_slow(JobBufs);
__global__ void k_build_blocks(JobBufs, const uint32_t *);
__global__ void k_scan_blocks(JobBufs);
__global__ void k_encode(JobBufs);

static __constant__ HuffTables s_tab;

constexpr uint32_t kLinks2Smem = 65536 * 2 + kLinkTile * 2 + kLinkTile + 64 + 2048;
constexpr uint32_t kPathSmem = kPathTile * 4 * 3;
constexpr uint32_t kChainSmem = kChainChunkTiles * kPathHead * 8;
constexpr uint32_t kChain2Max = 200 * 1024;

__global__ void __launch_bounds__(128) k_shard_entry(JobBufs jb, uint32_t S, uint32_t E, uint2 *out)
{
    const uint32_t c = blockIdx.x * blockDim.x + threadIdx.x;
    if (c >= kShardCand) return;
    const uint32_t te = jb.info->tail_entry;
    uint32_t spec_total = jb.info->n_mid_syms, spec_exit = te;
    if (te < E) { const uint32_t v = jb.nxt[te]; spec_total += (v >> 16) & 0xffu; spec_exit = te + (v & 0xffffu); }
    uint32_t p = S + c, cnt = 0, steps = 0;
    while (p < E) {
        const uint32_t idx = jb.symidx[p];
        if (idx) {
            const uint32_t k = jb.tile_symbase[p / kPathTile] + idx - 1;
            out[c] = make_uint2(spec_exit, cnt + spec_total - k);
            return;
        }
        const uint32_t v = jb.nxt[p];
        if ((v & 0xffffu) == 0 || ++steps > E) { atomicOr(&jb.info->error, 1u); return; }
        cnt += (v >> 16) & 0xffu;
        p += v & 0xffffu;
    }
    out[c] = make_uint2(p, cnt);
}

__global__ void __launch_bounds__(256) k_shard_hist(JobBufs jb, uint32_t *freq, ShardLoc *loc, uint32_t O, uint32_t n, uint32_t blo,
                                                    uint32_t bs)
{
    __shared__ uint32_t f[320];
    const uint32_t j = blockIdx.x, b = blo + j;
    for (uint32_t i = threadIdx.x; i < 320; i += blockDim.x) f[i] = 0;
    __syncthreads();
    const uint32_t lb = max(b * bs, O) - O;
    const uint32_t le = (uint32_t)min((uint64_t)(b + 1) * bs, (uint64_t)O + n) - O;
    for (uint32_t i = lb + threadIdx.x; i < le; i += blockDim.x) {
        const Sym s = jb.syms[i];
        if (s.dist == 0) atomicAdd(&f[s.lc], 1u);
        else {
            atomicAdd(&f[257 + s_tab.length_code[s.lc]], 1u);
            atomicAdd(&f[kLCodes + d_code(s_tab, s.dist - 1u)], 1u);
        }
    }
    __syncthreads();
    for (uint32_t i = threadIdx.x; i < 320; i += blockDim.x) freq[(size_t)j * 320 + i] = f[i];
    if (threadIdx.x == 0) {
        const Sym fs = jb.syms[lb], ls = jb.syms[le - 1];
        const uint32_t end = ls.pos + (ls.dist ? (uint32_t)ls.lc + 3u : 1u);
        loc[j] = ShardLoc{lb, le - lb, fs.pos, end, ls.pos, ls.dist == 0 ? 1u : 0u, {0, 0}};
        BlockDesc &bd = jb.blocks[j];
        bd.sym_begin = lb;
        bd.sym_count = le - lb;
        bd.in_start = fs.pos;
        bd.in_len = end - fs.pos;
        bd.last = 0;
        bd.have_window = fs.pos >= base_at(ls.pos + 1, jb.N);
    }
}

__global__ void __launch_bounds__(256) k_shard_piece(JobBufs jb, const uint32_t *freq, const uint32_t *xloc, const ShardLoc *loc,
                                                     uint32_t nloc, uint32_t holds, zb_shard_span *span)
{
    for (uint32_t j = threadIdx.x; j < nloc; j += blockDim.x) {
        BlockDesc &bd = jb.blocks[j];
        bool hf = true, hl = true;
        const uint32_t *f = freq + (size_t)j * 320;
        if (j == 0) { hf = holds & 1u; hl = holds & 2u; f = xloc; }
        else if (j + 1 == nloc) { hf = holds & 4u; hl = holds & 8u; f = xloc + 320; }
        shard_piece(bd, hf, hl, loc[j], f, f + kLCodes);
        if (bd.type == 0 && (uint64_t)bd.in_start + (uint16_t)bd.in_len > jb.N) atomicOr(&jb.info->error, 128u);
    }
    __syncthreads();
    if (threadIdx.x == 0) {
        zb_shard_span s{0, 0, 0, 0};
        for (uint32_t j = 0; j < nloc; j++) shard_span_add(s, jb.blocks[j]);
        *span = s;
    }
}

#define SCK(call)                                                           \
    do {                                                                    \
        cudaError_t e_ = (call);                                            \
        if (e_ != cudaSuccess) {                                            \
            snprintf(g_err, sizeof g_err, "%s: %s", #call, cudaGetErrorString(e_)); \
            return ZB_E_CUDA;                                               \
        }                                                                   \
    } while (0)

static int shard_param(const char *what)
{
    snprintf(g_err, sizeof g_err, "zb_shard: %s", what);
    return ZB_E_PARAM;
}

void Engine::shard_chain()
{
    JobBufs &jb = shard.jb;
    uint32_t *mark_cnt = reinterpret_cast<uint32_t *>(shard.gfn + (size_t)shard.chain_groups * kPathHead), *mark_list = mark_cnt + 4;
    cudaMemsetAsync(jb.tile_entry, 0xee, (size_t)shard.npt * 4, st);
    if (shard.chain2_smem <= kChain2Max) {
        k_path_groups<<<shard.chain_groups, 1024, shard.chainG * kPathHead * 8, st>>>(jb, shard.npt, shard.chainG, shard.gfn, mark_cnt);
        k_path_chain2<<<shard.chain_groups, 1024, shard.chain2_smem, st>>>(jb, shard.npt, shard.chainG, shard.gfn, mark_list, mark_cnt);
        k_path_mark<<<shard.npt, 1024, kPathSmem, st>>>(jb, mark_list, mark_cnt);
    } else {
        k_path_chain<<<1, 1024, kChainSmem, st>>>(jb, shard.npt, 0);
        k_path_mark<<<shard.npt, 1024, kPathSmem, st>>>(jb, nullptr, nullptr);
    }
}

int Engine::shard_parse(const void *src, size_t total, bool src_dev, size_t S, size_t E, int level, int strategy, uint32_t flags,
                        zb_shard_entry *table, uint32_t *adler)
{
    shard.phase = 0;
    const int mem_level = (flags >> 8) & 15u ? (int)((flags >> 8) & 15u) : 8;
    if (!table || !adler || (!src && total)) return shard_param("null argument");
    if ((flags & ~0xf00u) || !shard_params_ok(level, strategy, mem_level))
        return shard_param("levels 7..9, Z_DEFAULT_STRATEGY / Z_FILTERED / Z_FIXED, memLevel 1..9 only");
    if (total > kShardMaxInput || S > E || E > total || (S == E && total)) return shard_param("range out of bounds");
    SCK(cudaSetDevice(device));
    if (!shard.tables) {
        HuffTables t;
        init_tables(t);
        SCK(cudaMemcpyToSymbol(s_tab, &t, sizeof t));
        shard.tables = true;
    }
    const ShardStage stg = shard_stage((uint32_t)S, (uint32_t)E, (uint32_t)total);
    const uint32_t N = stg.end - stg.off, Sj = (uint32_t)S - stg.off, Ej = (uint32_t)E - stg.off;
    const size_t npad = (size_t)N + kPad;
    const uint32_t nmt = N / kMatchTile + 1, npt = Ej / kPathTile + 1;
    JobBufs &jb = shard.jb;
    memset(&jb, 0, sizeof jb);
    int rc;
    void *p;
#define RES(slot, bytes, field, type)                        \
    if ((rc = reserve(slot, bytes, &p)) != ZB_OK) return rc; \
    jb.field = static_cast<type>(p);
    RES(S_IN, npad + 16, in, const uint8_t *)
    RES(S_L, npad * 2, L, uint16_t *)
    RES(S_KEYS, npad * 2, keys, uint16_t *)
    RES(S_M, npad * 4, M, uint32_t *)
    RES(S_NXT, ((size_t)N + 16) * 4, nxt, uint32_t *)
    RES(S_PEXIT, ((size_t)N + 16) * 4, pexit, uint32_t *)
    RES(S_PCNT, ((size_t)N + 16) * 4, pcnt, uint32_t *)
    RES(S_SYMIDX, ((size_t)N + 16) * 4, symidx, uint32_t *)
    RES(S_PHEAD, (size_t)npt * kPathHead * 8, phead, uint2 *)
    RES(S_TENTRY, (size_t)npt * 4, tile_entry, uint32_t *)
    RES(S_TSYMB, (size_t)npt * 4, tile_symbase, uint32_t *)
    RES(S_MARKN, (size_t)npt + 16, mark_needed, uint8_t *)
    RES(S_LLIST, (size_t)npt * (kPathTile / kPathSub) * kLongPerSub * 4, long_list, uint32_t *)
    RES(S_LCNT, (size_t)npt * (kPathTile / kPathSub) * 4, long_cnt, uint32_t *)
    RES(S_TDIRTY, (size_t)nmt + 16, tile_dirty, uint8_t *)
    RES(S_SYMS, ((size_t)N + 64) * sizeof(Sym), syms, Sym *)
    RES(S_LLAST, (size_t)nmt * 65536 * 2, link_last, uint16_t *)
    RES(S_CSTATE, (size_t)(npt + 1) * 16, chain_state, uint4 *)
#undef RES
    shard.chainG = 16;
    while ((uint64_t)shard.chainG * shard.chainG < npt) shard.chainG += 8;
    shard.chain_groups = (npt + shard.chainG - 1) / shard.chainG;
    shard.chain2_smem = shard.chainG * kPathHead * 8 + shard.chain_groups * kPathHead * 16 + shard.chainG * 8;
    if ((rc = reserve(S_GFN, (size_t)shard.chain_groups * kPathHead * 16 + ((size_t)npt + 4) * 4, &p)) != ZB_OK) return rc;
    shard.gfn = static_cast<uint4 *>(p);
    void *d_ck;
    const size_t ck_bytes = ((size_t)N / 16384 + 16) * 8;
    if ((rc = reserve(S_CK, ck_bytes, &d_ck)) != ZB_OK) return rc;
    uint2 *d_table;
    if ((rc = reserve(S_SHARD, kShardCand * 8, &p)) != ZB_OK) return rc;
    if ((rc = stage(kShardCand * 8)) != ZB_OK) return rc;
    d_table = static_cast<uint2 *>(p);
    jb.N = N;
    jb.start = Sj;
    jb.tail_start = Ej;
    jb.nmt = nmt;
    jb.info = d_info;
    jb.level = (uint32_t)level;
    jb.strategy_fixed = strategy == 4;
    jb.slow_mode = 1;
    jb.sp = slow_params(level);
    jb.sp.filtered = strategy == 1;
    jb.wsize = kWSize;
    jb.cinfo = 7;
    jb.lp = level_params(level);
    jb.block_syms = (1u << (mem_level + 6)) - 1u;
    uint8_t *d_in = const_cast<uint8_t *>(jb.in);
    if (N) SCK(cudaMemcpyAsync(d_in, static_cast<const uint8_t *>(src) + stg.off, N, src_dev ? cudaMemcpyDeviceToDevice : cudaMemcpyHostToDevice, st));
    SCK(cudaMemsetAsync(d_in + N, 0, kPad, st));
    SCK(cudaMemsetAsync(d_info, 0, sizeof(JobInfo), st));
    SCK(cudaMemsetAsync(jb.tile_dirty, 1, nmt, st));
    SCK(cudaMemsetAsync(jb.M + N, 0, (size_t)kPad * 4, st));
    SCK(cudaMemsetAsync(jb.L + N, 0, (size_t)kPad * 2, st));
    SCK(launch_adler32(d_in + Sj, Ej - Sj, 1, d_ck, ck_bytes, d_check, st));
    if (Ej > Sj) {
        if (jb.sp.slow) {
            k_links2_roll<<<nmt, 1024, kLinks2Smem, st>>>(jb, 0);
            k_links_fix_roll<<<N / 256 + 1, 256, 0, st>>>(jb);
        } else {
            k_links2_std<<<nmt, 1024, kLinks2Smem, st>>>(jb, 0);
            k_links_fix_std<<<N / 256 + 1, 256, 0, st>>>(jb);
        }
        jb.match_sub = level >= 9 ? 24576u : level == 8 ? 4096u : 8192u;
        k_slow<<<(Ej + jb.match_sub - 1) / jb.match_sub, 1024, (kWSize + jb.match_sub + kSlowAhead) * 3, st>>>(jb);
        k_path_tiles<<<npt, 1024, kPathSmem, st>>>(jb);
        shard.npt = npt;
        shard_chain();
        k_shard_entry<<<(kShardCand + 127) / 128, 128, 0, st>>>(jb, Sj, Ej, d_table);
        SCK(cudaMemcpyAsync(h_stage, d_table, kShardCand * 8, cudaMemcpyDeviceToHost, st));
    }
    SCK(cudaMemcpyAsync(h_info, d_info, sizeof(JobInfo), cudaMemcpyDeviceToHost, st));
    SCK(cudaStreamSynchronize(st));
    SCK(cudaGetLastError());
    if (h_info->error) { snprintf(g_err, sizeof g_err, "engine error flags 0x%x (shard parse)", h_info->error); return ZB_E_INTERNAL; }
    uint32_t a = 1;
    SCK(cudaMemcpy(&a, d_check, 4, cudaMemcpyDeviceToHost));
    *adler = a;
    const uint2 *t = reinterpret_cast<const uint2 *>(h_stage);
    for (uint32_t c = 0; c < kShardCand; c++)
        table[c] = Ej > Sj ? zb_shard_entry{t[c].x + stg.off, t[c].y} : zb_shard_entry{(uint32_t)S + c, 0u};
    shard.off = stg.off; shard.S = Sj; shard.E = Ej; shard.total = (uint32_t)total;
    shard.bs = jb.block_syms; shard.npt = npt;
    shard.phase = 1;
    return ZB_OK;
}

int Engine::shard_symbols(uint32_t entry, uint32_t sym_offset, zb_shard_edge *first, zb_shard_edge *last)
{
    if (shard.phase != 1) { shard.phase = 0; return shard_param("zb_shard_symbols needs zb_shard_parse first"); }
    shard.phase = 0;
    JobBufs &jb = shard.jb;
    const uint32_t off = shard.off, Sj = shard.S, Ej = shard.E;
    if (!first || !last) return shard_param("null argument");
    if (entry < Sj + off || entry - (Sj + off) >= kShardCand || entry > shard.total) return shard_param("entry outside the entry table");
    SCK(cudaSetDevice(device));
    const uint32_t ej = entry - off;
    uint32_t n = 0;
    if (ej < Ej) {
        if (ej != Sj) { jb.start = ej; shard_chain(); }
        k_emit_slow<<<(Ej + 255) / 256, 256, 0, st>>>(jb);
        SCK(cudaMemcpyAsync(h_info, d_info, sizeof(JobInfo), cudaMemcpyDeviceToHost, st));
        SCK(cudaStreamSynchronize(st));
        n = h_info->n_mid_syms;
        if (h_info->tail_entry < Ej) {
            k_tail_slow<<<1, 32, 0, st>>>(jb);
            SCK(cudaMemcpyAsync(h_info, d_info, sizeof(JobInfo), cudaMemcpyDeviceToHost, st));
            SCK(cudaStreamSynchronize(st));
            n = h_info->n_syms;
        }
        SCK(cudaGetLastError());
        if (h_info->error) { snprintf(g_err, sizeof g_err, "engine error flags 0x%x (shard symbols)", h_info->error); return ZB_E_INTERNAL; }
    }
    if (n > kShardMaxInput - sym_offset) return shard_param("symbol offset out of range");
    const uint32_t bs = shard.bs;
    shard.O = sym_offset;
    shard.n = n;
    shard.is_last = Ej + off == shard.total;
    shard.blo = sym_offset / bs;
    shard.nloc = n ? (sym_offset + n - 1) / bs - shard.blo + 1 : 0;
    const uint32_t nb = shard.nloc + 1;
    int rc;
    void *p;
    if ((rc = reserve(S_BLOCKS, (size_t)nb * sizeof(BlockDesc), &p)) != ZB_OK) return rc;
    jb.blocks = static_cast<BlockDesc *>(p);
    if ((rc = reserve(S_FREQ, (size_t)nb * 320 * 4, &p)) != ZB_OK) return rc;
    uint32_t *d_freq = static_cast<uint32_t *>(p);
    if ((rc = reserve(S_SHARD, (size_t)nb * sizeof(ShardLoc) + 2 * 320 * 4 + 64, &p)) != ZB_OK) return rc;
    ShardLoc *d_loc = static_cast<ShardLoc *>(p);
    ShardLoc lo{}, hi{};
    if (shard.nloc) {
        k_shard_hist<<<shard.nloc, 256, 0, st>>>(jb, d_freq, d_loc, sym_offset, n, shard.blo, bs);
        SCK(cudaMemcpyAsync(&lo, d_loc, sizeof lo, cudaMemcpyDeviceToHost, st));
        SCK(cudaMemcpyAsync(&hi, d_loc + shard.nloc - 1, sizeof hi, cudaMemcpyDeviceToHost, st));
        SCK(cudaMemcpyAsync(shard.freq_lo, d_freq, 320 * 4, cudaMemcpyDeviceToHost, st));
        SCK(cudaMemcpyAsync(shard.freq_hi, d_freq + (size_t)(shard.nloc - 1) * 320, 320 * 4, cudaMemcpyDeviceToHost, st));
        SCK(cudaStreamSynchronize(st));
        SCK(cudaGetLastError());
    }
    auto edge = [&](const ShardLoc &l, const uint32_t *f, uint32_t j, zb_shard_edge &e) {
        memset(&e, 0, sizeof e);
        e.sym_offset = sym_offset;
        e.sym_count = n;
        e.is_last = shard.is_last;
        if (!shard.nloc) { e.block = kShardNone; return; }
        e.block = shard.blo + j;
        e.nsyms = l.count;
        e.first_pos = l.first_pos + off; e.end_pos = l.end_pos + off; e.last_pos = l.last_pos + off; e.last_lit = l.last_lit;
        e.flush_base = base_at(e.last_pos + 1, shard.total);
        memcpy(e.freq, f, sizeof e.freq);
    };
    edge(lo, shard.freq_lo, 0, *first);
    edge(hi, shard.freq_hi, shard.nloc ? shard.nloc - 1 : 0, *last);
    shard.phase = 2;
    return ZB_OK;
}

int Engine::shard_size(const zb_shard_edge *all, size_t n, zb_shard_span *span)
{
    if (shard.phase != 2) { shard.phase = 0; return shard_param("zb_shard_size needs zb_shard_symbols first"); }
    shard.phase = 0;
    if (!all || !span) return shard_param("null argument");
    JobBufs &jb = shard.jb;
    const uint32_t bs = shard.bs, off = shard.off, O = shard.O, ns = shard.n;
    ShardPlan pl;
    if (shard_plan(all, n, shard.total, bs, pl) != 0) return shard_param("edge records do not add up");
    uint32_t lo = 0;
    const uint32_t nl = shard_blocks(O, ns, shard.is_last, pl.fin, bs, lo);
    if (nl < shard.nloc || nl > shard.nloc + 1 || (shard.nloc && lo != shard.blo)) return shard_param("edge records do not add up");
    *span = zb_shard_span{0, 0, 0, 0};
    SCK(cudaSetDevice(device));
    void *p;
    int rc;
    if ((rc = reserve(S_FREQ, (size_t)(shard.nloc + 1) * 320 * 4, &p)) != ZB_OK) return rc;
    uint32_t *d_freq = static_cast<uint32_t *>(p);
    if ((rc = reserve(S_SHARD, (size_t)(shard.nloc + 1) * sizeof(ShardLoc) + 2 * 320 * 4 + 64, &p)) != ZB_OK) return rc;
    ShardLoc *d_loc = static_cast<ShardLoc *>(p);
    uint32_t *d_xloc = reinterpret_cast<uint32_t *>(d_loc + shard.nloc + 1);
    zb_shard_span *d_span = reinterpret_cast<zb_shard_span *>(d_xloc + 2 * 320);
    if (nl > shard.nloc) {
        const ShardLoc e{ns, 0, 0, 0, 0, 0, {0, 0}};
        SCK(cudaMemcpyAsync(d_loc + shard.nloc, &e, sizeof e, cudaMemcpyHostToDevice, st));
        SCK(cudaMemsetAsync(d_freq + (size_t)shard.nloc * 320, 0, 320 * 4, st));
        if (shard.nloc) memset(shard.freq_hi, 0, sizeof shard.freq_hi);
        else { memset(shard.freq_lo, 0, sizeof shard.freq_lo); memset(shard.freq_hi, 0, sizeof shard.freq_hi); }
        shard.nloc = nl;
        shard.blo = lo;
    }
    const uint32_t nloc = shard.nloc;
    if (!nloc) { shard.phase = 3; shard.span = *span; return ZB_OK; }
    uint32_t holds = 0;
    static thread_local BlockDesc hb;
    static thread_local ShardBlock m;
    for (int k = 0; k < 2; k++) {
        const uint32_t j = k == 0 ? 0 : nloc - 1, b = shard.blo + j;
        if (shard_merge(all, n, pl, b, bs, shard.total, m) != 0) return shard_param("edge records do not add up");
        SCK(cudaMemcpyAsync(&hb, jb.blocks + j, sizeof hb, cudaMemcpyDeviceToHost, st));
        SCK(cudaStreamSynchronize(st));
        hb.sym_count = m.nsyms;
        hb.in_start = m.in_start >= off ? m.in_start - off : 0u;
        hb.in_len = m.in_end - m.in_start;
        hb.last = b == pl.fin;
        hb.have_window = m.in_start >= m.flush_base;
        SCK(cudaMemcpyAsync(jb.blocks + j, &hb, sizeof hb, cudaMemcpyHostToDevice, st));
        SCK(cudaMemcpyAsync(d_freq + (size_t)j * 320, m.freq, 320 * 4, cudaMemcpyHostToDevice, st));
        SCK(cudaStreamSynchronize(st));
        holds |= (shard_holds_first(O, ns, shard.is_last, pl, b, bs) ? 1u : 0u) << (2 * k);
        holds |= (shard_holds_last(O, ns, shard.is_last, pl, b, bs) ? 2u : 0u) << (2 * k);
    }
    SCK(cudaMemcpyAsync(d_xloc, shard.freq_lo, 320 * 4, cudaMemcpyHostToDevice, st));
    SCK(cudaMemcpyAsync(d_xloc + 320, shard.freq_hi, 320 * 4, cudaMemcpyHostToDevice, st));
    SCK(cudaMemcpyAsync(&d_info->n_blocks, &nloc, 4, cudaMemcpyHostToDevice, st));
    k_build_blocks<<<nloc, 32, 0, st>>>(jb, d_freq);
    k_shard_piece<<<1, 256, 0, st>>>(jb, d_freq, d_xloc, d_loc, nloc, holds, d_span);
    SCK(cudaMemcpyAsync(span, d_span, sizeof *span, cudaMemcpyDeviceToHost, st));
    SCK(cudaMemcpyAsync(h_info, d_info, sizeof(JobInfo), cudaMemcpyDeviceToHost, st));
    SCK(cudaStreamSynchronize(st));
    SCK(cudaGetLastError());
    if (h_info->error) { snprintf(g_err, sizeof g_err, "engine error flags 0x%x (shard size)", h_info->error); return ZB_E_INTERNAL; }
    shard.span = *span;
    shard.phase = 3;
    return ZB_OK;
}

int Engine::shard_encode(uint64_t bit_offset, void *dst, size_t cap, bool dst_dev, uint64_t *bytes)
{
    if (shard.phase != 3) { shard.phase = 0; return shard_param("zb_shard_encode needs zb_shard_size first"); }
    if (!bytes) { shard.phase = 0; return shard_param("null argument"); }
    JobBufs &jb = shard.jb;
    const uint32_t prime = (uint32_t)(bit_offset & 7u);
    const uint64_t end = shard_span_end(shard.span, prime), need = (end + 7) >> 3;
    *bytes = need;
    if (cap < need || (!dst && need)) return ZB_E_BUF;
    shard.phase = 0;
    if (!need) return ZB_OK;
    SCK(cudaSetDevice(device));
    if (!shard.nloc) {
        if (dst_dev) SCK(cudaMemset(dst, 0, need)); else memset(dst, 0, need);
        return ZB_OK;
    }
    void *p;
    int rc;
    const size_t out_cap = (need + 64) & ~(size_t)15;
    if ((rc = reserve(S_OUT, out_cap + 16, &p)) != ZB_OK) return rc;
    jb.out = static_cast<uint8_t *>(p);
    jb.out_cap = out_cap;
    jb.prime_bits = prime;
    jb.wrap = 0;
    jb.hdr_len = 0;
    jb.not_last = 0;
    SCK(cudaMemsetAsync(jb.out, 0, out_cap, st));
    k_scan_blocks<<<1, 256, 0, st>>>(jb);
    k_encode<<<shard.nloc, 1024, 0, st>>>(jb);
    SCK(cudaMemcpyAsync(h_info, d_info, sizeof(JobInfo), cudaMemcpyDeviceToHost, st));
    SCK(cudaStreamSynchronize(st));
    SCK(cudaGetLastError());
    if (h_info->error || h_info->total_bits != end) {
        snprintf(g_err, sizeof g_err, "engine error flags 0x%x, %llu bits for a span of %llu (shard encode)", h_info->error,
                 (unsigned long long)h_info->total_bits, (unsigned long long)end);
        return ZB_E_INTERNAL;
    }
    SCK(cudaMemcpyAsync(dst, jb.out, need, dst_dev ? cudaMemcpyDeviceToDevice : cudaMemcpyDeviceToHost, st));
    SCK(cudaStreamSynchronize(st));
    return ZB_OK;
}

}

extern "C" {

struct zb_engine { zb::Engine e; };

int zb_shard_parse(zb_engine *z, const void *src, size_t total_len, int src_on_device, size_t range_begin, size_t range_end, int level,
                   int strategy, uint32_t flags, zb_shard_entry *table, uint32_t *adler)
{
    if (!z) return ZB_E_NODEVICE;
    return z->e.shard_parse(src, total_len, src_on_device != 0, range_begin, range_end, level, strategy, flags, table, adler);
}

int zb_shard_symbols(zb_engine *z, uint32_t entry, uint32_t sym_offset, zb_shard_edge *first, zb_shard_edge *last)
{
    if (!z) return ZB_E_NODEVICE;
    return z->e.shard_symbols(entry, sym_offset, first, last);
}

int zb_shard_size(zb_engine *z, const zb_shard_edge *all, size_t n, zb_shard_span *span)
{
    if (!z) return ZB_E_NODEVICE;
    return z->e.shard_size(all, n, span);
}

int zb_shard_encode(zb_engine *z, uint64_t bit_offset, void *dst, size_t cap, int dst_on_device, uint64_t *bytes)
{
    if (!z) return ZB_E_NODEVICE;
    return z->e.shard_encode(bit_offset, dst, cap, dst_on_device != 0, bytes);
}

}
```

Baseline: 1.645.

## Make iterative path/holes refresh incremental and shrink path tile shared memory

Later iterations no longer recompute all hole bits. Long-match intervals are stored directly in the long list, old and new intervals are collected, and only the touched words are updated and diffed, replacing full-array holes/cmp passes. The serial chain kernel can now resume near the dirty range and stop early once a tile entry matches its previous value, shifting symbol bases for the rest. k_path_tiles aliases nx/ex and uses 16-bit counts to halve shared memory, allowing two blocks per SM. These changes add atomics, more bookkeeping state and a consistency check flag in exchange for skipping work.

```diff
diff --git a/zlib_rs_b200/csrc/zb_engine.cu b/zlib_rs_b200/csrc/zb_engine.cu
--- a/zlib_rs_b200/csrc/zb_engine.cu
+++ b/zlib_rs_b200/csrc/zb_engine.cu
@@ -33,7 +33,7 @@
 __global__ void k_skip_walk(JobBufs);
 __global__ void k_nxt(JobBufs);
 __global__ void k_path_tiles(JobBufs);
-__global__ void k_path_chain(JobBufs, uint32_t, uint32_t);
+__global__ void k_path_chain(JobBufs, uint32_t, uint32_t, uint32_t, uint32_t *, uint32_t *);
 __global__ void k_path_groups(JobBufs, uint32_t, uint32_t, uint4 *, uint32_t *);
 __global__ void k_path_chain2(JobBufs, uint32_t, uint32_t, const uint4 *, uint32_t *, uint32_t *);
 __global__ void k_path_mark(JobBufs, const uint32_t *, const uint32_t *);
@@ -41,6 +41,8 @@
 __global__ void k_emit(JobBufs);
 __global__ void k_holes(JobBufs, uint32_t);
 __global__ void k_holes_cmp(JobBufs, uint32_t, uint32_t);
+__global__ void k_holes_clear(JobBufs, uint32_t);
+__global__ void k_holes_words(JobBufs);
 __global__ void k_tail(JobBufs);
 __global__ void k_block_hist(JobBufs, uint32_t *);
 __global__ void k_build_blocks(JobBufs, const uint32_t *);
@@ -116,7 +118,8 @@
     CK(cudaFuncSetAttribute(k_links2_std, cudaFuncAttributeMaxDynamicSharedMemorySize, kLinks2SmemBytes));
     CK(cudaFuncSetAttribute(k_links2_roll, cudaFuncAttributeMaxDynamicSharedMemorySize, kLinks2SmemBytes));
     CK(cudaFuncSetAttribute(k_slow, cudaFuncAttributeMaxDynamicSharedMemorySize, kSlowSmemBytes));
-    CK(cudaFuncSetAttribute(k_path_tiles, cudaFuncAttributeMaxDynamicSharedMemorySize, kPathSmemBytes));
+    CK(cudaFuncSetAttribute(k_path_tiles, cudaFuncAttributeMaxDynamicSharedMemorySize, kPathTilesSmem));
+    CK(cudaFuncSetAttribute(k_path_tiles, cudaFuncAttributePreferredSharedMemoryCarveout, cudaSharedmemCarveoutMaxShared));
     CK(cudaFuncSetAttribute(k_path_mark, cudaFuncAttributeMaxDynamicSharedMemorySize, kPathSmemBytes));
     CK(cudaFuncSetAttribute(k_path_chain, cudaFuncAttributeMaxDynamicSharedMemorySize, kChainSmemBytes));
     CK(cudaFuncSetAttribute(k_path_groups, cudaFuncAttributeMaxDynamicSharedMemorySize, kChain2MaxSmem));
@@ -275,7 +278,7 @@
     RES(S_TSYMB, (size_t)npt * 4, tile_symbase, uint32_t *)
     RES(S_MARKN, (size_t)npt + 16, mark_needed, uint8_t *)
     const uint32_t nlists = npt * (kPathTile / kPathSub);
-    RES(S_LLIST, (size_t)nlists * kLongPerSub * 4, long_list, uint32_t *)
+    RES(S_LLIST, (size_t)nlists * kLongPerSub * 8, long_list, uint2 *)
     RES(S_LCNT, (size_t)nlists * 4, long_cnt, uint32_t *)
     RES(S_TDIRTY, 2 * ((size_t)nmt + 16), tile_dirty, uint8_t *)
     jb.skip_fall = jb.tile_dirty + nmt + 16;
@@ -295,16 +298,15 @@
     uint4 *d_gfn = static_cast<uint4 *>(p);
     uint32_t *d_mark_cnt = reinterpret_cast<uint32_t *>(d_gfn + (size_t)chain_groups * kPathHead);
     uint32_t *d_mark_list = d_mark_cnt + 4;
-    auto launch_chain = [&](uint32_t first_tile) {
-        if (chain2) {
+    auto launch_chain = [&](uint32_t first_tile, bool resume) {
+        if (chain2 && !resume) {
             k_path_groups<<<chain_groups, 1024, chainG * kPathHead * 8, st>>>(jb, npt, chainG, d_gfn, d_mark_cnt);
             k_path_chain2<<<chain_groups, 1024, chain2_smem, st>>>(jb, npt, chainG, d_gfn, d_mark_list, d_mark_cnt);
             launches++;
-        } else k_path_chain<<<1, 1024, kChainSmemBytes, st>>>(jb, npt, first_tile);
+        } else k_path_chain<<<1, 1024, kChainSmemBytes, st>>>(jb, npt, first_tile, resume ? 1u : 0u, d_mark_list, d_mark_cnt);
     };
     auto launch_mark = [&](uint32_t grid) {
-        if (chain2) k_path_mark<<<grid < npt ? grid : npt, 1024, kPathSmemBytes, st>>>(jb, d_mark_list, d_mark_cnt);
-        else k_path_mark<<<npt, 1024, kPathSmemBytes, st>>>(jb, nullptr, nullptr);
+        k_path_mark<<<grid < npt ? grid : npt, 1024, kPathSmemBytes, st>>>(jb, d_mark_list, d_mark_cnt);
     };
     uint32_t *d_lists;
     const uint32_t max_list = N / 512 + 2;
@@ -313,6 +315,14 @@
     RES(S_HDIFF, (size_t)nwords * 8, hdiff, uint32_t *)
     jb.hdiff_words = nwords;
     RES(S_HCOARSE, (size_t)(N >> 10) + 16, hcoarse, uint8_t *)
+    const uint32_t nflag = nwords / 32 + 1;
+    jb.hiv_half = nlists * kLongPerSub;
+    const size_t hiv_off = ((size_t)nwords * 2 + nflag + 4 + 1) & ~(size_t)1;
+    RES(S_HWORDS, hiv_off * 4 + (size_t)jb.hiv_half * 16, hclr, uint32_t *)
+    jb.hword_flag = jb.hclr + nwords;
+    jb.hcnt = jb.hword_flag + nflag;
+    jb.hword_list = jb.hcnt + 4;
+    jb.hiv = reinterpret_cast<uint2 *>(jb.hclr + hiv_off);
     RES(S_MCHG, (((size_t)N >> 8) + 16) * 4 + 64, mchg, uint8_t *)
     RES(S_BLOCKS, (size_t)max_blocks * sizeof(BlockDesc), blocks, BlockDesc *)
     RES(S_BBASE, (size_t)max_blocks * 4, block_base, uint32_t *)
@@ -455,6 +465,7 @@
         } else {
             CK(cudaMemsetAsync(jb.holes, 0, (size_t)nwords * 4, st));
             CK(cudaMemsetAsync(jb.holes_new, 0, (size_t)nwords * 4, st));
+            CK(cudaMemsetAsync(jb.hclr, 0, ((size_t)nwords + nflag + 4) * 4, st));
             CK(cudaMemsetAsync(jb.tile_dirty, 1, nmt, st));
             CK(cudaMemsetAsync(jb.skip_fall, 0, nmt, st));
             CK(cudaMemsetAsync(jb.tile_entry, 0xee, (size_t)npt * 4, st));
@@ -492,8 +503,8 @@
                     pend(1, 1);
                     if (profile) phase_ms[11] = phase_ms[1];
                     pbegin();
-                    k_path_tiles<<<npt, 1024, kPathSmemBytes, st>>>(jb);
-                    launch_chain(0);
+                    k_path_tiles<<<npt, 1024, kPathTilesSmem, st>>>(jb);
+                    launch_chain(0, false);
                     launch_mark(npt);
                     pend(3, 3);
                     pbegin();
@@ -543,6 +554,7 @@
                     const uint32_t msmem = (kWSize + jb.match_sub + 512) + (kWSize + jb.match_sub) * 2 +
                                            (iters > 1 ? ((kWSize + jb.match_sub) / 32 + 1) * 4 * 4 + 8192 : 64);
                     jb.use_bucket_map = iters > 1;
+                    jb.hole_words = iters > 1;
                     pbegin();
                     k_match<<<nsub, mthreads, msmem, st>>>(jb);
                     pend(1, 1);
@@ -551,13 +563,19 @@
                     k_nxt<<<n_ptiles * (kPathTile / 1024), 1024, 0, st>>>(jb);
                     pend(2, 1);
                     pbegin();
-                    k_path_tiles<<<n_ptiles, 1024, kPathSmemBytes, st>>>(jb);
-                    launch_chain(first_ptile);
+                    k_path_tiles<<<n_ptiles, 1024, kPathTilesSmem, st>>>(jb);
+                    launch_chain(first_ptile, iters > 1 && h_info->last_ptile - first_ptile < kChainResumeTiles);
                     launch_mark(iters == 1 ? npt : 2 * n_ptiles + 16);
                     pend(3, 3);
                     pbegin();
-                    k_holes<<<(nlists * kLongPerSub + 255) / 256, 256, 0, st>>>(jb, nlists);
-                    k_holes_cmp<<<(nwords + 255) / 256, 256, 0, st>>>(jb, nwords, nmt);
+                    if (iters == 1) {
+                        k_holes<<<(nlists * kLongPerSub + 255) / 256, 256, 0, st>>>(jb, nlists);
+                        k_holes_cmp<<<(nwords + 255) / 256, 256, 0, st>>>(jb, nwords, nmt);
+                    } else {
+                        const uint32_t ncl = (uint32_t)device_sm_count();
+                        k_holes_clear<<<n_dirty > ncl ? n_dirty : ncl, 256, 0, st>>>(jb, n_dirty);
+                        k_holes_words<<<device_sm_count(), 256, 0, st>>>(jb);
+                    }
                     pend(4, 2);
                     launches += 7;
                     k_iter_lists<<<1, 1024, 0, st>>>(jb, d_lists, d_lists + nmt + 8, npt);
diff --git a/zlib_rs_b200/csrc/zb_engine_internal.h b/zlib_rs_b200/csrc/zb_engine_internal.h
--- a/zlib_rs_b200/csrc/zb_engine_internal.h
+++ b/zlib_rs_b200/csrc/zb_engine_internal.h
@@ -27,6 +27,7 @@
        S_ZIPPAY,
        S_ZIPOUT,
        S_ZIPTAB,
+       S_HWORDS,
        S_COUNT };
 
 struct ShardState {
@@ -90,7 +91,7 @@
 };
 
 struct Engine {
-    static constexpr int kSlots = 49;
+    static constexpr int kSlots = 50;
     struct Buf { void *p = nullptr; size_t cap = 0; };
     int device = -1;
     cudaStream_t st = nullptr, st2 = nullptr;
diff --git a/zlib_rs_b200/csrc/zb_kernels.cu b/zlib_rs_b200/csrc/zb_kernels.cu
--- a/zlib_rs_b200/csrc/zb_kernels.cu
+++ b/zlib_rs_b200/csrc/zb_kernels.cu
@@ -723,7 +723,8 @@
 }
 
 constexpr uint32_t kStuck = 0x80000000u;
-__device__ __forceinline__ void path_subtile(const uint32_t *nx, uint32_t *ex, uint32_t *cn, uint32_t s0, uint32_t s1, uint32_t lane)
+template <class CN>
+__device__ __forceinline__ void path_subtile(const uint32_t *nx, uint32_t *ex, CN *cn, uint32_t s0, uint32_t s1, uint32_t lane)
 {
     for (int32_t b = (int32_t)s1 - 32; b >= (int32_t)s0; b -= 32) {
         const uint32_t p = (uint32_t)b + lane;
@@ -741,7 +742,7 @@
         }
         if (!(t & kStuck) && t < s1) { c += cn[t]; t = ex[t]; }
         ex[p] = t;
-        cn[p] = c;
+        cn[p] = (CN)c;
         __syncwarp();
     }
 }
@@ -768,12 +769,12 @@
     }
 }
 
-__global__ void __launch_bounds__(1024) k_path_tiles(JobBufs jb)
+__global__ void __launch_bounds__(1024, 2) k_path_tiles(JobBufs jb)
 {
     extern __shared__ __align__(16) uint8_t smem[];
     uint32_t *nx = reinterpret_cast<uint32_t *>(smem);
-    uint32_t *ex = nx + kPathTile;
-    uint32_t *cn = ex + kPathTile;
+    uint32_t *ex = nx;
+    uint16_t *cn = reinterpret_cast<uint16_t *>(nx + kPathTile);
     const uint32_t tile = jb.nxt_list ? jb.nxt_list[blockIdx.x] : blockIdx.x;
     const uint32_t tbeg = tile * kPathTile;
     if (!path_tile_dirty(jb, tile)) return;
@@ -804,31 +805,39 @@
 }
 
 constexpr uint32_t kChainChunk = kChainChunkTiles;
-__global__ void __launch_bounds__(1024) k_path_chain(JobBufs jb, uint32_t ntiles, uint32_t first_tile)
+__global__ void __launch_bounds__(1024) k_path_chain(JobBufs jb, uint32_t ntiles, uint32_t first_tile, uint32_t resume,
+                                                       uint32_t *mark_list, uint32_t *mark_cnt)
 {
     extern __shared__ __align__(16) uint8_t smem[];
     uint2 *hd = reinterpret_cast<uint2 *>(smem);
-    __shared__ uint32_t s_e, s_base, s_done, s_tail;
-    __shared__ uint32_t c_entry[kChainChunk], c_base[kChainChunk];
+    __shared__ uint32_t s_e, s_base, s_done, s_tail, s_stop, s_nt;
+    __shared__ uint32_t c_entry[kChainChunk], c_base[kChainChunk], c_old[kChainChunk];
+    const uint32_t last_dirty = resume ? jb.info->last_ptile : 0xffffffffu;
     if (threadIdx.x == 0) {
         if (first_tile == 0) { s_e = jb.start; s_base = 0; s_done = jb.tail_start == 0; s_tail = jb.start; }
         else { const uint4 v = jb.chain_state[first_tile]; s_e = v.x; s_base = v.y; s_done = v.z; s_tail = v.w; }
+        s_stop = ntiles;
+        if (mark_list) *mark_cnt = 0;
     }
     for (uint32_t t = threadIdx.x; t < first_tile; t += blockDim.x) jb.mark_needed[t] = 0;
     __syncthreads();
-    for (uint32_t c0 = first_tile; c0 < ntiles; c0 += kChainChunk) {
-        const uint32_t nt = min(kChainChunk, ntiles - c0);
+    for (uint32_t c0 = first_tile, nt; c0 < ntiles && s_stop == ntiles; c0 += nt) {
+        nt = min(resume && c0 == first_tile ? 32u : kChainChunk, ntiles - c0);
         for (uint32_t i = threadIdx.x; i < nt * kPathHead; i += blockDim.x) hd[i] = jb.phead[(size_t)c0 * kPathHead + i];
+        if (resume) for (uint32_t k = threadIdx.x; k < nt; k += blockDim.x) c_old[k] = jb.tile_entry[c0 + k];
         __syncthreads();
         if (threadIdx.x == 0) {
             uint32_t e = s_e, base = s_base;
             bool done = s_done != 0;
             uint32_t tail_entry = s_tail;
-            for (uint32_t k = 0; k < nt; k++) {
+            uint32_t k = 0;
+            for (; k < nt; k++) {
                 const uint32_t tbeg = (c0 + k) * kPathTile, tend = tbeg + kPathTile;
+                const bool enter = !(done || e >= tend || e >= jb.tail_start);
+                if (c0 + k > last_dirty && enter && e == c_old[k]) { s_stop = c0 + k; break; }
                 jb.chain_state[c0 + k] = make_uint4(e, base, done ? 1u : 0u, tail_entry);
                 c_base[k] = base;
-                if (done || e >= tend || e >= jb.tail_start) { c_entry[k] = 0xffffffffu; continue; }
+                if (!enter) { c_entry[k] = 0xffffffffu; continue; }
                 c_entry[k] = e;
                 uint32_t x, c;
                 if (e - tbeg < kPathHead) { const uint2 v = hd[k * kPathHead + (e - tbeg)]; x = v.x; c = v.y; }
@@ -837,16 +846,30 @@
                 if (x & kStuck) { tail_entry = x & ~kStuck; done = true; }
                 else e = x;
             }
-            s_e = e; s_base = base; s_done = done; s_tail = tail_entry;
-        }
-        __syncthreads();
-        for (uint32_t k = threadIdx.x; k < nt; k += blockDim.x) {
+            s_e = e; s_base = base; s_done = done; s_tail = tail_entry; s_nt = k;
+        }
+        __syncthreads();
+        for (uint32_t k = threadIdx.x; k < s_nt; k += blockDim.x) {
             const uint32_t t = c0 + k;
             jb.tile_symbase[t] = c_base[k];
-            jb.mark_needed[t] = (jb.tile_entry[t] != c_entry[k]) || path_tile_dirty(jb, t);
+            const bool mn = (jb.tile_entry[t] != c_entry[k]) || path_tile_dirty(jb, t);
+            jb.mark_needed[t] = mn;
             jb.tile_entry[t] = c_entry[k];
-        }
-        __syncthreads();
+            if (mn && mark_list) mark_list[atomicAdd(mark_cnt, 1u)] = t;
+        }
+        __syncthreads();
+    }
+    const uint32_t stop = s_stop;
+    if (stop < ntiles) {
+        const uint32_t delta = s_base - jb.tile_symbase[stop];
+        __syncthreads();
+        for (uint32_t t = stop + threadIdx.x; t < ntiles; t += blockDim.x) {
+            jb.tile_symbase[t] += delta;
+            jb.chain_state[t].y += delta;
+            jb.mark_needed[t] = 0;
+        }
+        if (threadIdx.x == 0) jb.info->n_mid_syms += delta;
+        return;
     }
     if (threadIdx.x == 0) {
         uint32_t tail_entry = s_tail;
@@ -864,7 +887,7 @@
 {
     for (uint32_t k = 0; k < nt; k++) {
         const uint32_t tbeg = (t0 + k) * kPathTile, tend = tbeg + kPathTile;
-        if (OUT) c_base[k] = s.base;
+        if (OUT) { c_base[k] = s.base; jb.chain_state[t0 + k] = make_uint4(s.e, s.base, s.done, s.tail); }
         if (s.done || s.e >= tend || s.e >= jb.tail_start) { if (OUT) c_entry[k] = 0xffffffffu; continue; }
         if (OUT) c_entry[k] = s.e;
         uint32_t x, c;
@@ -958,6 +981,24 @@
         jb.mark_needed[t] = mn;
         jb.tile_entry[t] = c_entry[k];
         if (mn) mark_list[atomicAdd(mark_cnt, 1u)] = t;
+    }
+}
+
+__device__ __forceinline__ uint2 long_interior(const JobBufs &jb, uint32_t p, uint32_t v)
+{
+    const uint32_t delta = v & 0xffffu;
+    const uint32_t len = jb.lp.early_exit ? delta : ((v & kNxtLong258) ? 258u : 257u);
+    const uint32_t pos = p + delta - len;
+    return make_uint2(pos + 1, pos + len - 1);
+}
+
+__device__ __forceinline__ void holes_or(uint32_t *bits, uint2 iv)
+{
+    for (uint32_t y0 = iv.x; y0 < iv.y;) {
+        const uint32_t w = y0 >> 5, lo = y0 & 31;
+        const uint32_t n = min(32u - lo, iv.y - y0);
+        atomicOr(&bits[w], (n == 32 ? 0xffffffffu : ((1u << n) - 1u)) << lo);
+        y0 += n;
     }
 }
 
@@ -975,7 +1016,14 @@
         const uint32_t tbeg = tile * kPathTile;
         if (!jb.mark_needed[tile]) continue;
         const uint32_t entry = jb.tile_entry[tile];
-        if (threadIdx.x < nsub) jb.long_cnt[tile * nsub + threadIdx.x] = 0;
+        if (threadIdx.x < nsub) {
+            const uint32_t sl = tile * nsub + threadIdx.x, n = jb.long_cnt[sl];
+            if (jb.hole_words && n) {
+                const uint32_t o = atomicAdd(&jb.hcnt[1], n);
+                for (uint32_t k = 0; k < n; k++) jb.hiv[o + k] = jb.long_list[(size_t)sl * kLongPerSub + k];
+            }
+            jb.long_cnt[sl] = 0;
+        }
         if (entry == 0xffffffffu) {
             for (uint32_t i = threadIdx.x; i < kPathTile; i += blockDim.x)
                 if (tbeg + i < jb.tail_start) jb.symidx[tbeg + i] = 0;
@@ -1007,12 +1055,12 @@
             if (p != 0xffffffffu) {
                 uint32_t idx = sub_base[s], nlong = 0;
                 const uint32_t s1 = (s + 1) * kPathSub;
-                uint32_t *ll = jb.long_list + (size_t)(tile * nsub + s) * kLongPerSub;
+                uint2 *ll = jb.long_list + (size_t)(tile * nsub + s) * kLongPerSub;
                 while (p < s1) {
                     const uint32_t v = nx[p];
                     if (v & kNxtTail) break;
                     if (v & kNxtLong) {
-                        if (nlong < kLongPerSub) ll[nlong++] = tbeg + p;
+                        if (nlong < kLongPerSub) ll[nlong++] = long_interior(jb, tbeg + p, v);
                         else atomicOr(&jb.info->error, 32u);
                     }
                     ex[p] = idx + 1;
@@ -1020,6 +1068,10 @@
                     p += v & 0xffffu;
                 }
                 jb.long_cnt[tile * nsub + s] = nlong;
+                if (jb.hole_words && nlong) {
+                    const uint32_t o = jb.hiv_half + atomicAdd(&jb.hcnt[2], nlong);
+                    for (uint32_t k = 0; k < nlong; k++) jb.hiv[o + k] = ll[k];
+                }
             }
         }
         __syncthreads();
@@ -1041,18 +1093,70 @@
     }
     const uint32_t list = t / kLongPerSub, slot = t % kLongPerSub;
     if (list >= nlists || slot >= jb.long_cnt[list]) return;
-    const uint32_t p = jb.long_list[(size_t)list * kLongPerSub + slot];
-    const uint32_t v = jb.nxt[p], delta = v & 0xffffu;
-    const uint32_t len = jb.lp.early_exit ? delta : ((v & kNxtLong258) ? 258u : 257u);
-    const uint32_t pos = p + delta - len;
-    uint32_t y0 = pos + 1, y1 = pos + len - 1;
-    uint32_t *hn = jb.holes_new;
-    while (y0 < y1) {
-        const uint32_t w = y0 >> 5, lo = y0 & 31;
-        const uint32_t n = min(32u - lo, y1 - y0);
-        const uint32_t mask = (n == 32 ? 0xffffffffu : ((1u << n) - 1u)) << lo;
-        atomicOr(&hn[w], mask);
-        y0 += n;
+    holes_or(jb.holes_new, jb.long_list[(size_t)list * kLongPerSub + slot]);
+}
+
+__global__ void __launch_bounds__(256) k_holes_clear(JobBufs jb, uint32_t ntiles)
+{
+    const uint32_t tid = threadIdx.x;
+    if (blockIdx.x == 0 && tid == 0) jb.info->holes_changed = 0;
+    {
+        const uint32_t n0 = jb.hcnt[1], n = n0 + jb.hcnt[2];
+        for (uint32_t i = blockIdx.x * blockDim.x + tid; i < n * 16; i += gridDim.x * blockDim.x) {
+            const uint32_t j = i >> 4;
+            const uint2 iv = jb.hiv[j < n0 ? j : jb.hiv_half + j - n0];
+            const uint32_t w = (iv.x >> 5) + (i & 15);
+            if (iv.x >= iv.y || w > (iv.y - 1) >> 5) continue;
+            if ((i & 15) == 0) atomicAdd(&jb.hcnt[3], j < n0 ? iv.x - iv.y : iv.y - iv.x);
+            const uint32_t y0 = max(iv.x, w * 32), y1 = min(iv.y, w * 32 + 32), nb = y1 - y0;
+            atomicOr(&(j < n0 ? jb.hclr : jb.holes_new)[w], (nb == 32 ? 0xffffffffu : ((1u << nb) - 1u)) << (y0 & 31));
+            if (!(atomicOr(&jb.hword_flag[w >> 5], 1u << (w & 31)) & (1u << (w & 31)))) jb.hword_list[atomicAdd(&jb.hcnt[0], 1u)] = w;
+        }
+    }
+    if (blockIdx.x >= ntiles) return;
+    const uint32_t tile = jb.skip_list[blockIdx.x];
+    if (tid == 0) jb.tile_dirty[tile] = 0;
+    uint4 *bm = reinterpret_cast<uint4 *>(jb.bucket_map + (size_t)tile * 2048);
+    for (uint32_t i = tid; i < 512; i += blockDim.x) bm[i] = make_uint4(0, 0, 0, 0);
+    constexpr uint32_t wpt = kMatchTile / 32;
+    for (uint32_t i = tid; i < wpt; i += blockDim.x) {
+        const uint32_t w = tile * wpt + i;
+        if (w < jb.hdiff_words) { jb.hdiff[w] = 0; jb.hdiff[jb.hdiff_words + w] = 0; }
+    }
+    for (uint32_t i = tile * (kMatchTile >> 10) + tid; i < min((tile + 1) * (kMatchTile >> 10), (jb.N >> 10) + 16); i += blockDim.x)
+        jb.hcoarse[i] = 0;
+    for (uint32_t i = tile * (kMatchTile >> 8) + tid; i < min((tile + 1) * (kMatchTile >> 8), (jb.N >> 8) + 16); i += blockDim.x)
+        reinterpret_cast<uint32_t *>(jb.mchg)[i] = 0;
+}
+
+__global__ void __launch_bounds__(256) k_holes_words(JobBufs jb)
+{
+    const uint32_t cnt = jb.hcnt[0];
+    for (uint32_t i = blockIdx.x * blockDim.x + threadIdx.x; i < cnt; i += gridDim.x * blockDim.x) {
+        const uint32_t w = jb.hword_list[i];
+        const uint32_t a = jb.holes[w], b = (a & ~jb.hclr[w]) | jb.holes_new[w];
+        jb.hclr[w] = 0;
+        jb.holes_new[w] = 0;
+        jb.hword_flag[w >> 5] = 0;
+        if (a == b) continue;
+        atomicAdd(&jb.hcnt[3], (uint32_t)__popc(a) - (uint32_t)__popc(b));
+        jb.hdiff[w] = b & ~a;
+        jb.hdiff[jb.hdiff_words + w] = a & ~b;
+        jb.hcoarse[w >> 5] = 1;
+        const uint32_t t = (w * 32) / kMatchTile;
+        jb.info->holes_changed = 1u;
+        jb.tile_dirty[t] = 1;
+        if (t + 1 < jb.nmt) jb.tile_dirty[t + 1] = 1;
+        jb.holes[w] = b;
+        uint32_t *bm = jb.bucket_map + (size_t)t * 2048;
+        for (uint32_t diff = a ^ b; diff; diff &= diff - 1) {
+            const uint32_t y = w * 32 + (__ffs(diff) - 1);
+            if (y + 4 <= jb.N) {
+                const uint8_t *q = jb.in + y;
+                const uint32_t h = hash_u32((uint32_t)q[0] | ((uint32_t)q[1] << 8) | ((uint32_t)q[2] << 16) | ((uint32_t)q[3] << 24));
+                atomicOr(&bm[h >> 5], 1u << (h & 31));
+            }
+        }
     }
 }
 
@@ -1145,10 +1249,18 @@
         }
         __syncthreads();
         if (tid == 0) {
-            if (which) { jb.info->n_ptiles = base; jb.info->first_ptile = s_first == 0xffffffffu ? 0u : s_first; }
+            if (which) {
+                jb.info->n_ptiles = base;
+                jb.info->first_ptile = s_first == 0xffffffffu ? 0u : s_first;
+                jb.info->last_ptile = base ? out[base - 1] : 0u;
+            }
             else jb.info->n_dirty = base;
         }
         if (tid == 0 && base == 0) out[0] = 0;
+    }
+    if (jb.hcnt && tid < 4) {
+        if (tid == 3 && jb.hcnt[3]) atomicOr(&jb.info->error, 256u);
+        jb.hcnt[tid] = 0;
     }
 }
 
diff --git a/zlib_rs_b200/csrc/zb_kernels.cuh b/zlib_rs_b200/csrc/zb_kernels.cuh
--- a/zlib_rs_b200/csrc/zb_kernels.cuh
+++ b/zlib_rs_b200/csrc/zb_kernels.cuh
@@ -15,6 +15,7 @@
 constexpr uint32_t kPathSub = 256;
 constexpr uint32_t kLongPerSub = 4;
 constexpr uint32_t kPathHead = 64;
+constexpr uint32_t kPathTilesSmem = kPathTile * 6;
 constexpr uint32_t kChainChunkTiles = 320;
 constexpr uint32_t kNxtTail = 0x80000000u;
 constexpr uint32_t kNxtLong = 0x40000000u;
@@ -24,6 +25,7 @@
 constexpr uint32_t kSkipSlice = 4096;
 constexpr uint32_t kSkipWalkHops = 256;
 constexpr uint32_t kSkipWalkTiles = 32;
+constexpr uint32_t kChainResumeTiles = 48;
 
 __device__ __forceinline__ uint32_t sld_u8(uint32_t a) { uint32_t v; asm volatile("ld.shared.u8 %0, [%1];" : "=r"(v) : "r"(a)); return v; }
 __device__ __forceinline__ uint32_t sld_u16(uint32_t a) { uint32_t v; asm volatile("ld.shared.u16 %0, [%1];" : "=r"(v) : "r"(a)); return v; }
@@ -40,7 +42,7 @@
     uint32_t n_syms;
     uint32_t final_base;
     uint32_t holes_changed;
-    uint32_t n_dirty, n_ptiles, first_ptile;
+    uint32_t n_dirty, n_ptiles, first_ptile, last_ptile;
     uint32_t n_blocks;
     uint32_t data_type;
     uint32_t error;
@@ -91,8 +93,15 @@
     uint32_t match_sub;
     uint32_t nmt;
     uint8_t *mark_needed;
-    uint32_t *long_list;
+    uint2 *long_list;
     uint32_t *long_cnt;
+    uint32_t hole_words;
+    uint32_t *hclr;
+    uint32_t *hword_flag;
+    uint32_t *hcnt;
+    uint32_t *hword_list;
+    uint2 *hiv;
+    uint32_t hiv_half;
     SlowParams sp;
     uint32_t slow_mode;
     uint16_t *link_last;
diff --git a/zlib_rs_b200/csrc/zb_shard.cu b/zlib_rs_b200/csrc/zb_shard.cu
--- a/zlib_rs_b200/csrc/zb_shard.cu
+++ b/zlib_rs_b200/csrc/zb_shard.cu
@@ -12,7 +12,7 @@
 __global__ void k_links_fix_std(JobBufs);
 __global__ void k_links_fix_roll(JobBufs);
 __global__ void k_path_tiles(JobBufs);
-__global__ void k_path_chain(JobBufs, uint32_t, uint32_t);
+__global__ void k_path_chain(JobBufs, uint32_t, uint32_t, uint32_t, uint32_t *, uint32_t *);
 __global__ void k_path_groups(JobBufs, uint32_t, uint32_t, uint4 *, uint32_t *);
 __global__ void k_path_chain2(JobBufs, uint32_t, uint32_t, const uint4 *, uint32_t *, uint32_t *);
 __global__ void k_path_mark(JobBufs, const uint32_t *, const uint32_t *);
@@ -130,7 +130,7 @@
         k_path_chain2<<<shard.chain_groups, 1024, shard.chain2_smem, st>>>(jb, shard.npt, shard.chainG, shard.gfn, mark_list, mark_cnt);
         k_path_mark<<<shard.npt, 1024, kPathSmem, st>>>(jb, mark_list, mark_cnt);
     } else {
-        k_path_chain<<<1, 1024, kChainSmem, st>>>(jb, shard.npt, 0);
+        k_path_chain<<<1, 1024, kChainSmem, st>>>(jb, shard.npt, 0, 0, nullptr, nullptr);
         k_path_mark<<<shard.npt, 1024, kPathSmem, st>>>(jb, nullptr, nullptr);
     }
 }
@@ -174,7 +174,7 @@
     RES(S_TENTRY, (size_t)npt * 4, tile_entry, uint32_t *)
     RES(S_TSYMB, (size_t)npt * 4, tile_symbase, uint32_t *)
     RES(S_MARKN, (size_t)npt + 16, mark_needed, uint8_t *)
-    RES(S_LLIST, (size_t)npt * (kPathTile / kPathSub) * kLongPerSub * 4, long_list, uint32_t *)
+    RES(S_LLIST, (size_t)npt * (kPathTile / kPathSub) * kLongPerSub * 8, long_list, uint2 *)
     RES(S_LCNT, (size_t)npt * (kPathTile / kPathSub) * 4, long_cnt, uint32_t *)
     RES(S_TDIRTY, (size_t)nmt + 16, tile_dirty, uint8_t *)
     RES(S_SYMS, ((size_t)N + 64) * sizeof(Sym), syms, Sym *)
@@ -226,7 +226,7 @@
         }
         jb.match_sub = level >= 9 ? 24576u : level == 8 ? 4096u : 8192u;
         k_slow<<<(Ej + jb.match_sub - 1) / jb.match_sub, 1024, (kWSize + jb.match_sub + kSlowAhead) * 3, st>>>(jb);
-        k_path_tiles<<<npt, 1024, kPathSmem, st>>>(jb);
+        k_path_tiles<<<npt, 1024, kPathTilesSmem, st>>>(jb);
         shard.npt = npt;
         shard_chain();
         k_shard_entry<<<(kShardCand + 127) / 128, 128, 0, st>>>(jb, Sj, Ej, d_table);
```

Result: faster. 1.669 (median of 6 runs) (+1.5%).
